# MarcoMeter/endless-memory-gym

Measured on AMD Instinct MI355X. Metric: env steps/sec (aggregate), higher is better.
Workload: dtype u8; 1 GPU; MortarMayhem-Grid-v0, 65536 envs/GPU x 1 GPU, 84x84x3 obs (u8_xyc), same-step auto-reset, uniform random actions generated on device; env_id=MortarMayhem-Grid-v0, envs_per_gpu=65536, envs_total=65536, parallelism=env-sharded x1, no data-path collective

## Files before the change

### endless-memory-gym_amd/csrc/mg_api.hip

```cpp
#include <algorithm>
#include <chrono>
#include <cstddef>
#include <map>
#include <mutex>

#include "mg_family.hpp"
#include "mg_lab.hpp"
using mg::lab_env;

namespace mg {
static thread_local std::string g_last_error;
void set_error(const std::string& msg) { g_last_error = msg; }
}

struct mg_env {
    mg::Family* fam = nullptr;
    int device = 0;
    int num_envs = 0;
    int variant = 0, family = 0;
    bool started = false;
    std::string id;
    int obs_format = MG_OBS_U8_XYC;
    float* vec_dev = nullptr;
    float* vec_dev_caller = nullptr;
    int prof_stride = 0;
    struct Single {
        bool open = false;
        char *host = nullptr, *dev = nullptr;
        size_t bytes = 0;
        size_t o_action = 0, o_seed = 0, o_obs = 0, o_vec = 0, o_reward32 = 0, o_reward = 0, o_done = 0, o_gt32 = 0, o_gt = 0, o_ep_reward = 0,
               o_ep_length = 0, o_aux = 0, o_flag = 0;
        uint32_t ticket = 0;
    } single;
};

namespace {
constexpr size_t INFO_SIZE_MIN = offsetof(mg_info_buffers, final_obs_dev);
mg_info_buffers read_info(const mg_info_buffers* info) {
    mg_info_buffers ib;
    memset(&ib, 0, sizeof(ib));
    if (!info) return ib;
    const size_t sz = info->struct_size;
    constexpr size_t INFO_SIZE_MAX = sizeof(mg_info_buffers) + 16 * sizeof(void*);
    if (sz < INFO_SIZE_MIN || sz > INFO_SIZE_MAX || sz % sizeof(void*) != 0)
        throw std::runtime_error("mg_step: mg_info_buffers.struct_size = " + std::to_string(sz) + " is not a layout of include/memgym.h (" +
                                 std::to_string(sizeof(mg_info_buffers)) + " in this build); set it to sizeof(mg_info_buffers)");
    memcpy(&ib, info, sz < sizeof(ib) ? sz : sizeof(ib));
    ib.struct_size = sizeof(ib);
    return ib;
}

struct StateHeader {
    char magic[8];
    uint32_t version, num_envs;
    uint64_t payload, id_hash;
    uint8_t pad[32];
};
static_assert(sizeof(StateHeader) == 64, "state header is 64 bytes");
uint64_t fnv1a(const std::string& s) {
    uint64_t h = 1469598103934665603ull;
    for (unsigned char c : s) h = (h ^ c) * 1099511628211ull;
    return h;
}

struct DeviceGuard {
    int prev = -1;
    explicit DeviceGuard(int device) {
        MG_HIP(hipGetDevice(&prev));
        if (prev != device) MG_HIP(hipSetDevice(device));
        else prev = -1;
    }
    ~DeviceGuard() {
        if (prev >= 0) (void)hipSetDevice(prev);
    }
};

template <typename F>
int guarded(mg_env* env, F&& f) {
    try {
        if (!env || !env->fam) {
            mg::set_error("null handle");
            return -1;
        }
        DeviceGuard guard(env->device);
        f();
        return 0;
    } catch (const mg::OptionError& e) {
        mg::set_error(e.msg);
        return e.code;
    } catch (const std::exception& e) {
        mg::set_error(e.what());
        return -1;
    }
}
}

namespace {
mg::Family* make_family(int family, int variant, int n) {
    if (family == 0) return mg::make_mortar(variant, n);
    if (family == 1) return mg::make_spot(variant, n);
    return mg::make_mystery(variant, n);
}
void destroy_family(mg_env* e) {
    if (e->single.host) {
        if (e->vec_dev && e->vec_dev == (float*)(e->single.dev + e->single.o_vec)) e->vec_dev = e->vec_dev_caller;
        (void)hipHostFree(e->single.host);
        e->single = mg_env::Single();
    }
    delete e->fam;
    e->fam = nullptr;
}
size_t obs_bytes_of(int f) {
    const size_t elem = f == MG_OBS_F32_CYX ? 4 : ((f == MG_OBS_F16_CYX || f == MG_OBS_BF16_CYX) ? 2 : 1);
    return elem * 84 * 84 * 3;
}
}

extern "C" {

const char* mg_last_error(void) { return mg::g_last_error.c_str(); }

int mg_create(const char* env_id, int32_t num_envs, int device, mg_env** out) {
    try {
        if (!env_id || !out || num_envs < 1) {
            mg::set_error("mg_create: bad arguments");
            return -1;
        }
        DeviceGuard guard(device);
        std::string id(env_id);
        int family = -1, variant = 0;
        if (id == "MortarMayhem-Grid-v0") { family = 0; variant = 0; }
        else if (id == "MortarMayhem-v0") { family = 0; variant = 1; }
        else if (id == "Endless-MortarMayhem-v0") { family = 0; variant = 2; }
        else if (id == "MortarMayhemB-Grid-v0") { family = 0; variant = 3; }
        else if (id == "MortarMayhemB-v0") { family = 0; variant = 4; }
        else if (id == "Endless-SearingSpotlights-v0") { family = 1; variant = 1; }
        else if (id == "SearingSpotlights-v0") { family = 1; variant = 0; }
        else if (id == "MysteryPath-v0") { family = 2; variant = 0; }
        else if (id == "Endless-MysteryPath-v0") { family = 2; variant = 1; }
        else if (id == "MysteryPath-Grid-v0") { family = 2; variant = 2; }
        else {
            mg::set_error("mg_create: environment id not available in this build: " + id);
            return -5;
        }
        mg_env* e = new mg_env();
        e->device = device;
        e->num_envs = num_envs;
        e->id = id;
        e->family = family;
        e->variant = variant;
        try {
            e->fam = make_family(family, variant, num_envs);
        } catch (...) {
            delete e;
            throw;
        }
        *out = e;
        return 0;
    } catch (const std::exception& e) {
        mg::set_error(e.what());
        return -1;
    }
}

void mg_destroy(mg_env* env) {
    if (!env) return;
    int prev = -1;
    (void)hipGetDevice(&prev);
    (void)hipSetDevice(env->device);
    (void)hipDeviceSynchronize();
    destroy_family(env);
    delete env;
    if (prev >= 0) (void)hipSetDevice(prev);
}

int32_t mg_num_envs(const mg_env* env) { return env ? env->num_envs : 0; }
int32_t mg_action_dim(const mg_env* env) { return env ? env->fam->action_dim() : 0; }
int32_t mg_gt_dim(const mg_env* env) { return env ? env->fam->gt_dim() : 0; }
int32_t mg_vec_dim(const mg_env* env) { return env ? env->fam->vec_dim() : 0; }
int mg_bind_vector_obs(mg_env* env, float* vec_dev) {
    return guarded(env, [&] {
        if (env->fam->vec_dim() == 0 && vec_dev) throw std::runtime_error("mg_bind_vector_obs: this env id has no vector observation");
        env->vec_dev = env->vec_dev_caller = vec_dev;
        env->fam->bind_vector_obs(vec_dev);
    });
}
const char* mg_info_name(const mg_env* env, int k) { return env ? env->fam->info_name(k) : nullptr; }

int mg_set_option(mg_env* env, const char* key, const double* values, int n) {
    return guarded(env, [&] {
        if (!key || !values || n < 1) throw mg::OptionError{-3, "mg_set_option: bad arguments"};
        env->fam->set_option(key, values, n);
    });
}

int mg_set_option_set(mg_env* env, int set_id, const char* key, const double* values, int n) {
    return guarded(env, [&] {
        if (!key || !values || n < 1) throw mg::OptionError{-3, "mg_set_option_set: bad arguments"};
        if (set_id < 0 || set_id >= MG_MAX_OPTION_SETS) throw mg::OptionError{-3, "mg_set_option_set: set index out of range"};
        env->fam->set_option_set(set_id, key, values, n);
    });
}

int mg_bind_option_sets(mg_env* env, const int32_t* set_of_dev) {
    return guarded(env, [&] {
        env->fam->bind_option_sets(set_of_dev);
    });
}

int mg_set_capacity(mg_env* env, const char* what, int64_t value) {
    return guarded(env, [&] {
        if (!what) throw mg::OptionError{-3, "mg_set_capacity: NULL"};
        if (env->started) throw std::runtime_error("mg_set_capacity: before the first mg_reset / mg_set_state");
        env->fam->set_capacity(what, value);
    });
}
int64_t mg_capacity(mg_env* env, const char* what) {
    int64_t v = -1;
    const int rc = guarded(env, [&] {
        if (!what) throw mg::OptionError{-3, "mg_capacity: NULL"};
        v = env->fam->capacity(what);
    });
    return rc == 0 ? v : -1;
}

int mg_set_obs_format(mg_env* env, int format) {
    return guarded(env, [&] {
        if (format != MG_OBS_U8_XYC && format != MG_OBS_F32_CYX && format != MG_OBS_F16_CYX && format != MG_OBS_BF16_CYX)
            throw mg::OptionError{-3, "mg_set_obs_format: unknown format"};
        env->obs_format = env->fam->obs_format = format;
    });
}

size_t mg_obs_bytes(const mg_env* env) {
    if (!env) return 0;
    return obs_bytes_of(env->obs_format);
}

int mg_reset(mg_env* env, const int64_t* seeds_dev, const uint8_t* mask_dev, void* obs_dev, float* gt_dev, void* stream) {
    return guarded(env, [&] {
        if (!obs_dev) throw std::runtime_error("mg_reset: obs_dev is NULL");
        env->fam->reset(seeds_dev, mask_dev, obs_dev, gt_dev, (hipStream_t)stream);
        env->started = true;
    });
}

int mg_render(mg_env* env, void* obs_dev, void* stream) {
    return guarded(env, [&] {
        if (!obs_dev) throw std::runtime_error("mg_render: obs_dev is NULL");
        env->fam->raster_only(obs_dev, nullptr, (hipStream_t)stream);
    });
}

typedef uint32_t row_vec16 __attribute__((ext_vector_type(4)));
constexpr int COPY_CHUNK = 16;
__global__ __launch_bounds__(256) void copy_rows_kernel(const uint8_t* __restrict__ flags, const row_vec16* __restrict__ src, row_vec16* __restrict__ dst,
                                                      int n, int vec_per_row) {
    const int tid = threadIdx.x;
    for (int base = blockIdx.x * COPY_CHUNK; base < n; base += gridDim.x * COPY_CHUNK) {
        const int e = base + (tid & (COPY_CHUNK - 1));
        uint32_t m = (uint32_t)__builtin_amdgcn_readfirstlane((int)(uint32_t)__ballot(e < n && flags[e] != 0)) & ((1u << COPY_CHUNK) - 1u);
        while (m) {
            const size_t row = (size_t)(base + __builtin_ctz(m)) * (size_t)vec_per_row;
            m &= m - 1;
            for (int q0 = 0; q0 < vec_per_row; q0 += 6 * 256) {
                row_vec16 v[6];
#pragma unroll
                for (int k = 0; k < 6; ++k) {
                    const int q = q0 + tid + 256 * k;
                    if (q < vec_per_row) v[k] = src[row + q];
                }
#pragma unroll
                for (int k = 0; k < 6; ++k) {
                    const int q = q0 + tid + 256 * k;
                    if (q < vec_per_row) dst[row + q] = v[k];
                }
            }
        }
    }
}

namespace {
__global__ __launch_bounds__(256) void debug_stretch_kernel(const uint8_t* __restrict__ frames, uint8_t* __restrict__ out, int n) {
    const size_t total = (size_t)n * 336 * 336;
    for (size_t p = (size_t)blockIdx.x * blockDim.x + threadIdx.x; p < total; p += (size_t)gridDim.x * blockDim.x) {
        const int x = (int)(p % 336), y = (int)((p / 336) % 336);
        const size_t e = p / (336 * 336);
        const uint8_t* src = frames + e * MG_OBS_BYTES + ((size_t)(x >> 2) * 84 + (y >> 2)) * 3;
        uint8_t* dst = out + p * 3;
        dst[0] = src[0];
        dst[1] = src[1];
        dst[2] = src[2];
    }
}
}

int mg_render_debug(mg_env* env, uint8_t* rgb_dev, void* stream) {
    return guarded(env, [&] {
        if (!rgb_dev) throw std::runtime_error("mg_render_debug: rgb_dev is NULL");
        hipStream_t st = (hipStream_t)stream;
        uint8_t* frames = nullptr;
        MG_HIP(hipMalloc((void**)&frames, (size_t)env->num_envs * MG_OBS_BYTES));
        try {
            env->fam->sync_state();
            env->fam->raster_debug(frames, st);
            const size_t total = (size_t)env->num_envs * 336 * 336;
            const unsigned grid = (unsigned)std::min<size_t>((total + 255) / 256, 65536);
            hipLaunchKernelGGL(debug_stretch_kernel, dim3(grid), dim3(256), 0, st, frames, rgb_dev, env->num_envs);
            MG_HIP(hipGetLastError());
            MG_HIP(hipStreamSynchronize(st));
        } catch (...) {
            (void)hipFree(frames);
            throw;
        }
        MG_HIP(hipFree(frames));
    });
}

int mg_step(mg_env* env, const int32_t* actions_dev, void* obs_dev, float* reward_dev, uint8_t* done_dev, float* gt_dev,
            const mg_info_buffers* info, int autoreset, void* stream) {
    return guarded(env, [&] {
        if (!actions_dev || !obs_dev || !reward_dev || !done_dev) throw std::runtime_error("mg_step: NULL buffer");
        hipStream_t st = (hipStream_t)stream;
        const mg_info_buffers ib = read_info(info);
        mg::Family* f = env->fam;
        if (autoreset && ib.final_obs_dev && !(mg::sparse_masked_raster() && f->keeps_final_obs(st))) {
            f->step(actions_dev, obs_dev, reward_dev, done_dev, gt_dev, &ib, 0, st);
            if (mg::sparse_masked_raster()) {
                const int n = env->num_envs, vec_per_row = (int)(mg_obs_bytes(env) / 16);
                hipLaunchKernelGGL(copy_rows_kernel, dim3(std::min((n + COPY_CHUNK - 1) / COPY_CHUNK, 16384)), dim3(256), 0, st, done_dev, (const row_vec16*)obs_dev,
                                   (row_vec16*)ib.final_obs_dev, n, vec_per_row);
                MG_HIP(hipGetLastError());
            } else f->raster_only(ib.final_obs_dev, done_dev, st);
            f->reset(nullptr, done_dev, obs_dev, gt_dev, st);
        } else {
            f->step(actions_dev, obs_dev, reward_dev, done_dev, gt_dev, &ib, autoreset, st);
        }
        if (ib.gt64_dev) f->ground_truth64(ib.gt64_dev, st);
    });
}

int mg_ground_truth64(mg_env* env, double* gt64_dev, void* stream) {
    return guarded(env, [&] {
        if (!env->fam->gt_dim()) return;
        if (!gt64_dev) throw std::runtime_error("mg_ground_truth64: gt64_dev is NULL");
        env->fam->sync_state();
        env->fam->ground_truth64(gt64_dev, (hipStream_t)stream);
    });
}

}
namespace {
void single_wait(mg_env::Single& S, hipStream_t st, bool armed = false) {
    static bool use_flag = true;
    if (use_flag) {
        const uint32_t want = armed ? S.ticket : ++S.ticket;
        if (armed || hipStreamWriteValue32(st, S.dev + S.o_flag, want, 0) == hipSuccess) {
            volatile uint32_t* flag = (volatile uint32_t*)(S.host + S.o_flag);
            const auto t0 = std::chrono::steady_clock::now();
            for (uint32_t spins = 0;; ++spins) {
                if (__atomic_load_n(flag, __ATOMIC_ACQUIRE) == want) return;
                __builtin_ia32_pause();
                if ((spins & 1023u) == 1023u && std::chrono::steady_clock::now() - t0 > std::chrono::milliseconds(50)) break;
            }
        } else {
            (void)hipGetLastError();
            use_flag = false;
        }
    }
    MG_HIP(hipStreamSynchronize(st));
}
}
extern "C" {
int mg_single_open(mg_env* env, mg_single_io* io) {
    return guarded(env, [&] {
        if (!io || io->struct_size != sizeof(mg_single_io)) throw std::runtime_error("mg_single_open: set io->struct_size = sizeof(mg_single_io)");
        if (env->num_envs != 1) throw std::runtime_error("mg_single_open: the handle must hold exactly one instance");
        mg_env::Single& S = env->single;
        if (!S.open) {
            size_t o = 0;
            auto take = [&](size_t bytes) { const size_t at = o; o = (o + bytes + 255) & ~(size_t)255; return at; };
            S.o_action = take(8); S.o_seed = take(8);
            S.o_obs = take(84 * 84 * 3 * 4);
            S.o_vec = take(sizeof(float) * 256);
            S.o_reward32 = take(4); S.o_reward = take(8); S.o_done = take(1);
            S.o_gt32 = take(sizeof(float) * 8); S.o_gt = take(sizeof(double) * 8);
            S.o_ep_reward = take(8); S.o_ep_length = take(4); S.o_aux = take(sizeof(float) * MG_INFO_SLOTS * 64);
            S.o_flag = take(4);
            S.bytes = o;
            MG_HIP(hipHostMalloc((void**)&S.host, S.bytes, hipHostMallocMapped | hipHostMallocCoherent));
            memset(S.host, 0, S.bytes);
            MG_HIP(hipHostGetDevicePointer((void**)&S.dev, S.host, 0));
            S.open = true;
        }
        if (env->fam->vec_dim()) {
            env->vec_dev = (float*)(S.dev + S.o_vec);
            env->fam->bind_vector_obs(env->vec_dev);
        }
        io->obs = S.host + S.o_obs;
        io->vec = env->fam->vec_dim() ? (float*)(S.host + S.o_vec) : nullptr;
        io->reward = (double*)(S.host + S.o_reward);
        io->done = (uint8_t*)(S.host + S.o_done);
        io->gt = (double*)(S.host + S.o_gt);
        io->ep_reward = (double*)(S.host + S.o_ep_reward);
        io->ep_length = (int32_t*)(S.host + S.o_ep_length);
        for (int k = 0; k < MG_INFO_SLOTS; ++k) io->aux[k] = (float*)(S.host + S.o_aux + 256 * k);
    });
}

int mg_single_reset(mg_env* env, int64_t seed, int has_seed, void* stream) {
    return guarded(env, [&] {
        mg_env::Single& S = env->single;
        if (!S.open) throw std::runtime_error("mg_single_reset: mg_single_open first");
        hipStream_t st = (hipStream_t)stream;
        *(int64_t*)(S.host + S.o_seed) = seed;
        mg::Family* f = env->fam;
        f->reset(has_seed ? (const int64_t*)(S.dev + S.o_seed) : nullptr, nullptr, S.dev + S.o_obs, f->gt_dim() ? (float*)(S.dev + S.o_gt32) : nullptr, st);
        f->ground_truth64((double*)(S.dev + S.o_gt), st);
        env->started = true;
        single_wait(S, st);
    });
}

int mg_single_step(mg_env* env, int32_t a0, int32_t a1, void* stream) {
    int flags = 0;
    const int rc = guarded(env, [&] {
        mg_env::Single& S = env->single;
        if (!S.open) throw std::runtime_error("mg_single_step: mg_single_open first");
        hipStream_t st = (hipStream_t)stream;
        int32_t* act = (int32_t*)(S.host + S.o_action);
        act[0] = a0;
        act[1] = a1;
        mg_info_buffers ib;
        memset(&ib, 0, sizeof(ib));
        ib.struct_size = sizeof(ib);
        ib.ep_reward_dev = (double*)(S.dev + S.o_ep_reward);
        ib.ep_length_dev = (int32_t*)(S.dev + S.o_ep_length);
        for (int k = 0; k < MG_INFO_SLOTS; ++k) ib.aux_dev[k] = (float*)(S.dev + S.o_aux + 256 * k);
        ib.reward64_dev = (double*)(S.dev + S.o_reward);
        mg::Family* f = env->fam;
        const bool armed = f->arm_done_flag((uint32_t*)(S.dev + S.o_flag), S.ticket + 1);
        if (armed) ++S.ticket;
        f->step((const int32_t*)(S.dev + S.o_action), S.dev + S.o_obs, (float*)(S.dev + S.o_reward32), (uint8_t*)(S.dev + S.o_done),
                f->gt_dim() ? (float*)(S.dev + S.o_gt32) : nullptr, &ib, 0, st);
        f->ground_truth64((double*)(S.dev + S.o_gt), st);
        single_wait(S, st, armed);
        flags = f->peek_errors();
    });
    return rc != 0 ? rc : flags;
}

size_t mg_state_size(const mg_env* env) {
    if (!env) return 0;
    size_t t = sizeof(StateHeader);
    for (auto& b : env->fam->state_blobs()) t += b.second;
    return t;
}

int mg_get_state(mg_env* env, void* host_buf, size_t size) {
    return guarded(env, [&] {
        if (!host_buf || size < mg_state_size(env)) throw std::runtime_error("mg_get_state: buffer too small");
        MG_HIP(hipDeviceSynchronize());
        env->fam->sync_state();
        StateHeader h;
        memset(&h, 0, sizeof(h));
        memcpy(h.magic, "MGSTATE1", 8);
        h.version = MG_STATE_VERSION;
        h.num_envs = (uint32_t)env->num_envs;
        h.payload = mg_state_size(env) - sizeof(StateHeader);
        h.id_hash = fnv1a(env->id);
        memcpy(host_buf, &h, sizeof(h));
        char* p = (char*)host_buf + sizeof(StateHeader);
        for (auto& b : env->fam->state_blobs()) {
            MG_HIP(hipMemcpy(p, b.first, b.second, hipMemcpyDeviceToHost));
            p += b.second;
        }
    });
}

int mg_set_state(mg_env* env, const void* host_buf, size_t size) {
    return guarded(env, [&] {
        if (!host_buf || size < sizeof(StateHeader)) throw std::runtime_error("mg_set_state: buffer too small for a state header");
        StateHeader h;
        memcpy(&h, host_buf, sizeof(h));
        if (memcmp(h.magic, "MGSTATE1", 8) != 0) throw std::runtime_error("mg_set_state: not a memgym state blob (bad magic)");
        if (h.version != MG_STATE_VERSION)
            throw std::runtime_error("mg_set_state: state version " + std::to_string(h.version) + ", this library reads version " +
                                     std::to_string(MG_STATE_VERSION));
        if (h.id_hash != fnv1a(env->id)) throw std::runtime_error("mg_set_state: the blob belongs to another env id than " + env->id);
        if (h.num_envs != (uint32_t)env->num_envs)
            throw std::runtime_error("mg_set_state: the blob holds " + std::to_string(h.num_envs) + " instances, the handle " +
                                     std::to_string(env->num_envs));
        if (h.payload != mg_state_size(env) - sizeof(StateHeader) || size < mg_state_size(env))
            throw std::runtime_error("mg_set_state: payload size differs from this handle's state");
        MG_HIP(hipDeviceSynchronize());
        const char* p = (const char*)host_buf + sizeof(StateHeader);
        for (auto& b : env->fam->state_blobs()) {
            MG_HIP(hipMemcpy(b.first, p, b.second, hipMemcpyHostToDevice));
            p += b.second;
        }
        env->fam->on_state_loaded();
        env->started = true;
    });
}

int mg_set_profiling(mg_env* env, int on) {
    return guarded(env, [&] {
        env->prof_stride = on < 0 ? 0 : on;
        env->fam->prof.stride = env->prof_stride;
        env->fam->prof.count[0] = env->fam->prof.count[1] = 0;
    });
}

int mg_get_profile(mg_env* env, int kind, double* total_ms, int64_t* launches) {
    return guarded(env, [&] {
        if (kind < 0 || kind > 1 || !total_ms || !launches) throw std::runtime_error("mg_get_profile: bad arguments");
        env->fam->prof.collect(kind, total_ms, launches);
    });
}

int mg_poll_errors(mg_env* env, int* flags) {
    return guarded(env, [&] {
        if (!flags) throw std::runtime_error("mg_poll_errors: NULL");
        MG_HIP(hipDeviceSynchronize());
        *flags = env->fam->poll_errors();
    });
}

int mg_peek_errors(mg_env* env, int* flags) {
    return guarded(env, [&] {
        if (!flags) throw std::runtime_error("mg_peek_errors: NULL");
        *flags = env->fam->peek_errors();
    });
}

int mg_enable_peer_access(int device, int peer_device) {
    try {
        int prev = 0;
        MG_HIP(hipGetDevice(&prev));
        struct Restore {
            int d;
            ~Restore() { (void)hipSetDevice(d); }
        } restore{prev};
        if (device == peer_device) return 0;
        int can = 0;
        MG_HIP(hipDeviceCanAccessPeer(&can, device, peer_device));
        if (!can) {
            mg::set_error("device " + std::to_string(device) + " has no peer access to device " + std::to_string(peer_device));
            return -1;
        }
        MG_HIP(hipSetDevice(device));
        hipError_t e = hipDeviceEnablePeerAccess(peer_device, 0);
        if (e != hipSuccess && e != hipErrorPeerAccessAlreadyEnabled) {
            (void)hipGetLastError();
            mg::set_error(std::string("hipDeviceEnablePeerAccess: ") + hipGetErrorString(e));
            return -1;
        }
        (void)hipGetLastError();
        return 0;
    } catch (const std::exception& e) {
        mg::set_error(e.what());
        return -1;
    }
}

int mg_debug_counter(mg_env* env, const char* name, int64_t* value) {
    return guarded(env, [&] {
        if (!name || !value) throw std::runtime_error("mg_debug_counter: NULL");
        MG_HIP(hipDeviceSynchronize());
        if (!env->fam->debug_counter(name, value)) throw std::runtime_error(std::string("mg_debug_counter: no counter named ") + name + " for " + env->id);
    });
}

int mg_debug_rng(mg_env* env, int32_t i, uint64_t* out) {
    return guarded(env, [&] {
        if (i < 0 || i >= env->num_envs) throw std::runtime_error("mg_debug_rng: index out of range");
        MG_HIP(hipDeviceSynchronize());
        env->fam->sync_state();
        env->fam->debug_rng(i, out);
    });
}

}
```

### endless-memory-gym_amd/csrc/mg_family.hpp

```cpp
#pragma once
#include <hip/hip_runtime.h>

#include <cstdint>
#include <cstdio>
#include <cstring>
#include <stdexcept>
#include <string>
#include <vector>

#include "../../include/memgym.h"
#include "mg_lab.hpp"
#include "mg_device.hpp"

namespace mg {

void set_error(const std::string& msg);
static_assert(MG_MAX_OPTION_SETS == 8, "set_index() (mg_device.hpp) masks an instance's set index with 7");

#define MG_HIP(expr)                                                                                 \
    do {                                                                                             \
        hipError_t e_ = (expr);                                                                      \
        if (e_ != hipSuccess)                                                                        \
            throw std::runtime_error(std::string(#expr) + " failed: " + hipGetErrorString(e_));      \
    } while (0)

struct ErrorWord {
    int* host = nullptr;
    int* dev = nullptr;
    ErrorWord() {}
    ErrorWord(const ErrorWord&) = delete;
    ErrorWord& operator=(const ErrorWord&) = delete;
    ~ErrorWord() {
        if (host) (void)hipHostFree(host);
    }
    void alloc() {
        MG_HIP(hipHostMalloc((void**)&host, 64, hipHostMallocMapped | hipHostMallocCoherent));
        *host = 0;
        MG_HIP(hipHostGetDevicePointer((void**)&dev, host, 0));
    }
    int peek() const { return __atomic_load_n(host, __ATOMIC_ACQUIRE); }
    int take() { return __atomic_exchange_n(host, 0, __ATOMIC_ACQ_REL); }
};

#ifdef __HIPCC__
__device__ __forceinline__ void raise_error(int* err, int bit) {
    __hip_atomic_fetch_or(err, bit, __ATOMIC_RELAXED, __HIP_MEMORY_SCOPE_SYSTEM);
}
constexpr int ERR_QUEUE_OVERFLOW = 64;
__device__ __forceinline__ void queue_push(int* queue, int* counter, int cap, int value, int* err) {
    const int slot = atomicAdd(counter, 1);
    if (__builtin_expect(slot < cap, 1)) queue[slot] = value;
    else raise_error(err, ERR_QUEUE_OVERFLOW);
}
__device__ __forceinline__ int queue_count(const int* counter, int cap) {
    const int c = *counter;
    return c < cap ? c : cap;
}
#endif

template <typename T>
struct DevArray {
    T* p = nullptr;
    size_t n = 0;
    DevArray() {}
    DevArray(const DevArray&) = delete;
    DevArray& operator=(const DevArray&) = delete;
    ~DevArray() { release(); }
    void release() {
        if (p) (void)hipFree(p);
        p = nullptr;
        n = 0;
    }
    void alloc(size_t count, bool zero = true) {
        release();
        n = count;
        MG_HIP(hipMalloc((void**)&p, sizeof(T) * (count ? count : 1)));
        if (zero) MG_HIP(hipMemset(p, 0, sizeof(T) * (count ? count : 1)));
    }
    void upload(const std::vector<T>& v) {
        alloc(v.size(), false);
        MG_HIP(hipMemcpy(p, v.data(), sizeof(T) * v.size(), hipMemcpyHostToDevice));
    }
    size_t bytes() const { return sizeof(T) * n; }
};

struct RngStore {
    DevArray<uint64_t> s_hi, s_lo, i_hi, i_lo, buf;
    void alloc(size_t n) { s_hi.alloc(n); s_lo.alloc(n); i_hi.alloc(n); i_lo.alloc(n); buf.alloc(n); }
    RngSoA view() { return RngSoA{s_hi.p, s_lo.p, i_hi.p, i_lo.p, buf.p}; }
    void blobs(std::vector<std::pair<void*, size_t>>& v) {
        v.push_back({s_hi.p, s_hi.bytes()}); v.push_back({s_lo.p, s_lo.bytes()}); v.push_back({i_hi.p, i_hi.bytes()});
        v.push_back({i_lo.p, i_lo.bytes()}); v.push_back({buf.p, buf.bytes()});
    }
    void debug(int i, uint64_t out[6]) {
        uint64_t b;
        MG_HIP(hipMemcpy(&out[0], s_hi.p + i, 8, hipMemcpyDeviceToHost));
        MG_HIP(hipMemcpy(&out[1], s_lo.p + i, 8, hipMemcpyDeviceToHost));
        MG_HIP(hipMemcpy(&out[2], i_hi.p + i, 8, hipMemcpyDeviceToHost));
        MG_HIP(hipMemcpy(&out[3], i_lo.p + i, 8, hipMemcpyDeviceToHost));
        MG_HIP(hipMemcpy(&b, buf.p + i, 8, hipMemcpyDeviceToHost));
        out[4] = (b >> 32) & 1;
        out[5] = b & 0xFFFFFFFFull;
    }
};

struct OptListStore {
    DevArray<int32_t> ext;
    std::vector<int> host;
    int max(const OptList& l) const {
        int m = 0;
        if (!host.empty() || l.ext) {
            for (int x : host) m = x > m ? x : m;
            return m;
        }
        for (int k = 0; k < l.n && k < OPT_INLINE; ++k) {
            const int x = (int)((l.w[k >> 2] >> (8 * (k & 3))) & 0xFFu);
            m = x > m ? x : m;
        }
        return m;
    }
    void set(OptList& l, const std::vector<int>& v) {
        host = v;
        l.n = (int)v.size();
        for (int j = 0; j < OPT_INLINE / 4; ++j) l.w[j] = 0u;
        l.ext = nullptr;
        bool bytes = true;
        for (int x : v) bytes = bytes && x >= 0 && x <= 255;
        for (int k = 0; bytes && k < l.n && k < OPT_INLINE; ++k) l.w[k >> 2] |= (uint32_t)(v[k] & 0xFF) << (8 * (k & 3));
        if (l.n > OPT_INLINE || !bytes) {
            std::vector<int32_t> b(v.begin(), v.end());
            MG_HIP(hipDeviceSynchronize());
            ext.upload(b);
            l.ext = ext.p;
        }
    }
};

struct OptionError {
    int code;
    std::string msg;
};

struct KernelProfile {
    int stride = 0;
    uint64_t count[2] = {0, 0};
    bool live[2] = {false, false};
    std::vector<std::pair<hipEvent_t, hipEvent_t>> ev[2];
    void begin(int kind, hipStream_t s) {
        live[kind] = stride > 0 && (count[kind]++ % (uint64_t)stride) == 0;
        if (!live[kind]) return;
        hipEvent_t a, b;
        MG_HIP(hipEventCreate(&a));
        MG_HIP(hipEventCreate(&b));
        MG_HIP(hipEventRecord(a, s));
        ev[kind].push_back({a, b});
    }
    void end(int kind, hipStream_t s) {
        if (!live[kind]) return;
        MG_HIP(hipEventRecord(ev[kind].back().second, s));
    }
    void collect(int kind, double* ms, int64_t* launches) {
        double t = 0;
        for (auto& p : ev[kind]) {
            MG_HIP(hipEventSynchronize(p.second));
            float f = 0;
            MG_HIP(hipEventElapsedTime(&f, p.first, p.second));
            t += f;
            (void)hipEventDestroy(p.first);
            (void)hipEventDestroy(p.second);
        }
        *ms = t;
        *launches = (int64_t)ev[kind].size();
        ev[kind].clear();
    }
};

class Family {
   public:
    KernelProfile prof;
    void end_logic(hipStream_t s) { prof.end(0, s); }
    int obs_format = MG_OBS_U8_XYC;
    virtual ~Family() {}
    virtual int action_dim() const = 0;
    virtual int gt_dim() const = 0;
    virtual bool arm_done_flag(uint32_t* , uint32_t ) { return false; }
    virtual void set_capacity(const std::string& what, int64_t) { throw OptionError{-2, "this env id has no capacity named " + what}; }
    virtual int64_t capacity(const std::string& what) const { throw OptionError{-2, "this env id has no capacity named " + what}; }
    virtual int vec_dim() const { return 0; }
    virtual void bind_vector_obs(float* ) {}
    virtual const char* info_name(int k) const = 0;
    virtual void set_option(const std::string& key, const double* v, int n) = 0;
    virtual void set_option_set(int set, const std::string& key, const double* v, int n) {
        if (set != 0) throw OptionError{-3, "this env id has no per-instance option sets in this build (use one handle per option set)"};
        set_option(key, v, n);
    }
    virtual void bind_option_sets(const int32_t* set_of_dev) {
        if (set_of_dev) throw OptionError{-3, "this env id has no per-instance option sets in this build (use one handle per option set)"};
    }
    virtual void reset(const int64_t* seeds, const uint8_t* mask, void* obs, float* gt, hipStream_t s) = 0;
    virtual void step(const int32_t* actions, void* obs, float* reward, uint8_t* done, float* gt,
                      const mg_info_buffers* info, int autoreset, hipStream_t s) = 0;
    virtual void raster_only(void* obs, const uint8_t* only, hipStream_t s) = 0;
    virtual bool keeps_final_obs(hipStream_t ) { return false; }
    virtual void raster_debug(void* frames, hipStream_t s) = 0;
    virtual std::vector<std::pair<void*, size_t>> state_blobs() = 0;
    virtual void on_state_loaded() {}
    virtual void sync_state() {}
    virtual void debug_rng(int i, uint64_t out[6]) = 0;
    virtual void ground_truth64(double* , hipStream_t ) {}
    virtual int poll_errors() { return 0; }
    virtual int peek_errors() { return 0; }
    virtual bool debug_counter(const std::string& , int64_t* ) { return false; }
};

Family* make_mortar(int variant, int num_envs);
Family* make_spot(int endless, int num_envs);
Family* make_mystery(int variant, int num_envs);

inline int step_block(int shipped) {
    static const int forced = [] {
        const char* e = lab_env("MEMGYM_STEP_BLOCK");
        const int v = e ? atoi(e) : 0;
        return (v == 64 || v == 128 || v == 256) ? v : 0;
    }();
    return forced ? forced : shipped;
}

inline int to_int_checked(double v, const char* key) {
    int i = (int)v;
    if ((double)i != v) throw OptionError{-3, std::string("option ") + key + " must be integral"};
    return i;
}

}
```

### endless-memory-gym_amd/csrc/mg_mortar.hip

```cpp
#include <memory>

#include "mg_atlas_v1.hpp"
#include "mg_device.hpp"
#include "mg_family.hpp"
#include "mg_lab.hpp"
#include "mg_raster_v1.hpp"
#include "mg_stamps.hpp"

namespace mg {
using namespace v1;

enum { V_GRID = 0, V_FREE = 1, V_ENDLESS = 2 };

struct MortarParams {
    int variant, N, allowed, visual_feedback, max_steps, initial_count;
    int taskb;
    int cmd_cap;
    int arena_x0, tile;
    int radius, sprite_dim;
    int glyph_x0;
    int v_axis_i, v_diag_i;
    int off_lo, off_hi;
    double v_axis, v_diag;
    OptList command_count, show_dur, show_delay, expl_dur, expl_delay;
    double r_fail, r_succ, r_ep_succ, r_new;
};

struct __attribute__((aligned(16))) MortarState {
    int16_t ax, ay;
    int16_t disp_x, disp_y;
    uint8_t rot8 : 3;
    uint8_t disp_is_agent : 1;
    uint8_t tiles_on : 1;
    uint8_t disp_sprite;
    int8_t tx, ty;
    int8_t nx, ny;
    uint16_t num_cmds, cur_cmd;
    uint16_t vis_pos, vis_len, vis_base;
    uint16_t cmd_steps, verify_step;
    uint16_t show_dur, show_delay, expl_dur, expl_delay;
    uint8_t gx, gy;
    int32_t ep_len, t, total_completed;
    uint32_t dbg_pops;
    double ep_sum;
};
static_assert(sizeof(MortarState) == 64, "MortarState must be 64 bytes");

struct __attribute__((aligned(16))) MortarDesc {
    int16_t sx, sy;
    uint16_t tmpl;
    uint8_t sprite;
    uint8_t glyph;
    int16_t glyph_x0;
    int16_t ring_x, ring_y;
    uint8_t ring_on;
    uint8_t epoch;
};
static_assert(sizeof(MortarDesc) == 16, "MortarDesc must be 16 bytes");
constexpr int STAMP_SPRITE0 = 0, STAMP_GLYPH0 = 8, STAMP_RING = 18;

struct MortarComposer {
    typedef MortarDesc Desc;
    static __device__ __forceinline__ bool skip(const Desc* dp) { return dp->tmpl == 0xFFFF; }
    static __device__ __forceinline__ void compose(const Desc* dp, const RasterCtx& R) {
        const Desc& d = *dp;
#if defined(MG_LAB_NO_TEMPLATE) && MG_LAB_NO_TEMPLATE == 2
#elif defined(MG_LAB_NO_TEMPLATE)
        fill_clear(R);
#else
        fill_template(R, d.tmpl);
#endif
        __syncthreads();
#ifndef MG_LAB_NO_STAMPS
        if (d.sprite != 0xFF) stamp(R, STAMP_SPRITE0 + d.sprite, d.sx, d.sy);
        if (d.glyph < 9) {
            __syncthreads();
            stamp(R, STAMP_GLYPH0 + d.glyph, d.glyph_x0, d.glyph_x0);
        }
#endif
    }
};

struct MortarDebugComposer {
    typedef MortarDesc Desc;
    static __device__ __forceinline__ bool skip(const Desc*) { return false; }
    static __device__ __forceinline__ void compose(const Desc* dp, const RasterCtx& R) {
        MortarComposer::compose(dp, R);
        __syncthreads();
        if (dp->ring_on) stamp(R, STAMP_RING, dp->ring_x, dp->ring_y);
    }
};

constexpr uint32_t pack_deltas(const int (&v)[9]) {
    uint32_t m = 0;
    for (int c = 0; c < 9; ++c) m |= (uint32_t)(v[c] + 1) << (2 * c);
    return m;
}
constexpr int kDxHost[9] = {1, 0, -1, 0, 0, 1, 1, -1, -1}, kDyHost[9] = {0, 1, 0, -1, 0, 1, -1, 1, -1};
constexpr uint32_t CMD_DX_BITS = pack_deltas(kDxHost), CMD_DY_BITS = pack_deltas(kDyHost);
__device__ __forceinline__ int cmd_dx(int c) { return (int)((CMD_DX_BITS >> (2 * c)) & 3u) - 1; }
__device__ __forceinline__ int cmd_dy(int c) { return (int)((CMD_DY_BITS >> (2 * c)) & 3u) - 1; }

__device__ __forceinline__ int floordiv(int a, int b) {
    int q = a / b;
    return (a % b != 0 && a < 0) ? q - 1 : q;
}
__device__ __forceinline__ int mod6(int a) { return ((a % 6) + 6) % 6; }
__device__ __forceinline__ int round_haz(double v) { return v >= 0 ? (int)floor(v + 0.5) : -(int)floor(-v + 0.5); }

__constant__ int8_t kCmdOneHot[9] = {1, 4, 2, 3, 0, 5, 6, 7, 8};
constexpr int VEC_DIM = 180;

__device__ void mortar_reset(const MortarParams& P, MortarState& s, Pcg& g, uint8_t* cmds, MortarDesc& d, float* gt, float* vec) {
    if (s.disp_sprite != 0xFF && s.disp_is_agent) {
        s.disp_x = s.ax;
        s.disp_y = s.ay;
        s.disp_is_agent = 0;
    }
    int half = P.tile / 2;
    int tile_id = g.integers(0, P.N * P.N);
    int cx = P.arena_x0 + P.tile * (tile_id / P.N) + half;
    int cy = P.arena_x0 + P.tile * (tile_id % P.N) + half;
    if (P.variant == V_ENDLESS || (P.taskb && P.variant == V_FREE)) {
        cx += g.integers(P.off_lo, P.off_hi);
        cy += g.integers(P.off_lo, P.off_hi);
    }
    s.ax = (int16_t)cx;
    s.ay = (int16_t)cy;
    s.rot8 = 0;
    int nx = floordiv(cx - P.arena_x0, P.tile), ny = floordiv(cy - P.arena_x0, P.tile);
    s.nx = (int8_t)nx;
    s.ny = (int8_t)ny;
    s.gx = (uint8_t)nx;
    s.gy = (uint8_t)ny;

    int n;
    if (P.variant == V_ENDLESS) {
        n = P.initial_count;
        for (int i = 0; i < n; ++i) cmds[i] = (uint8_t)g.integers(0, P.allowed);
    } else {
        n = choice(g, P.command_count);
        int px = nx, py = ny;
        for (int i = 0; i < n; ++i) {
            uint32_t valid = 0;
#pragma unroll
            for (int c = 0; c < 9; ++c) {
                const int qx = px + cmd_dx(c), qy = py + cmd_dy(c);
                if (c < P.allowed && qx >= 0 && qx < P.N && qy >= 0 && qy < P.N) valid |= 1u << c;
            }
            const int pick = g.integers(0, __popc(valid));
            uint32_t m = valid;
            for (int k = 0; k < pick; ++k) m &= m - 1;
            const int c = __ffs(m) - 1;
            cmds[i] = (uint8_t)c;
            px += cmd_dx(c);
            py += cmd_dy(c);
        }
    }
    s.num_cmds = (uint16_t)n;
    if (P.taskb) {
        s.show_dur = s.show_delay = 0;
    } else {
        s.show_dur = (uint16_t)choice(g, P.show_dur);
        s.show_delay = (uint16_t)choice(g, P.show_delay);
    }
    s.vis_len = (uint16_t)(n * (s.show_dur + s.show_delay));
    s.vis_base = 0;
    s.vis_pos = 1;
    s.dbg_pops = 0;
    int first = cmds[0];
    uint8_t glyph = s.show_dur > 0 ? (uint8_t)first : (uint8_t)9;
    if (P.variant == V_ENDLESS) {
        s.tx = (int8_t)mod6(nx + cmd_dx(first));
        s.ty = (int8_t)mod6(ny + cmd_dy(first));
    } else {
        s.tx = (int8_t)(nx + cmd_dx(first));
        s.ty = (int8_t)(ny + cmd_dy(first));
    }
    s.cur_cmd = 0;
    s.cmd_steps = 0;
    s.verify_step = 0;
    s.total_completed = 0;
    s.tiles_on = 0;
    s.t = 0;
    s.ep_len = 0;
    s.ep_sum = 0.0;
    s.expl_dur = (uint16_t)choice(g, P.expl_dur);
    s.expl_delay = (uint16_t)choice(g, P.expl_delay);

    d.tmpl = 0;
    d.sprite = 0;
    d.sx = (int16_t)(cx - P.sprite_dim / 2);
    d.sy = (int16_t)(cy - P.sprite_dim / 2);
    d.glyph = glyph;
    if (gt) {
        gt[0] = (float)(s.tx / 5.0);
        gt[1] = (float)(s.ty / 5.0);
    }
    if (vec) {
        for (int k = 0; k < VEC_DIM; ++k) vec[k] = 0.0f;
        for (int c = 0; c < n && c < VEC_DIM / 9; ++c) vec[9 * c + kCmdOneHot[cmds[c]]] = 1.0f;
    }
}

struct MortarIO {
    MortarState* state;
    uint8_t* cmds;
    RngSoA rng;
    MortarDesc* desc;
    float* vec;
    int* err;
    const MortarParams* sets;
    const int32_t* set_of;
};
constexpr int ERR_CMD_OVERFLOW = 32;

template <bool PS>
__global__ __launch_bounds__(256) void mortar_reset_kernel(MortarParams P0, int n, MortarIO io, const int64_t* seeds,
                                                           const uint8_t* mask, float* gt) {
    int i = blockIdx.x * blockDim.x + threadIdx.x;
    if (i >= n) return;
    const MortarParams& P = PS ? io.sets[set_index(io.set_of, i)] : P0;
    MortarDesc d;
    memset(&d, 0, sizeof(d));
    d.glyph_x0 = (int16_t)P.glyph_x0;
    if (mask && !mask[i]) {
        d.tmpl = 0xFFFF;
        io.desc[i] = d;
        return;
    }
    Pcg g;
    if (seeds) g.seed((uint64_t)seeds[i]);
    else g.load(io.rng, i);
    MortarState s = io.state[i];
    mortar_reset(P, s, g, io.cmds + (size_t)i * P.cmd_cap, d, gt ? gt + 2 * i : nullptr, io.vec ? io.vec + (size_t)i * VEC_DIM : nullptr);
    io.state[i] = s;
    g.store(io.rng, i);
    io.desc[i] = d;
}

__global__ __launch_bounds__(256) void mortar_init_kernel(int n, MortarState* state) {
    int i = blockIdx.x * blockDim.x + threadIdx.x;
    if (i >= n) return;
    MortarState s;
    memset(&s, 0, sizeof(s));
    s.disp_sprite = 0xFF;
    state[i] = s;
}

struct MortarStepArgs {
    MortarParams P;
    int n;
    MortarIO io;
    const int32_t* actions;
    float* reward_out;
    uint8_t* done_out;
    float* gt;
    mg_info_buffers info;
    int autoreset;
    MortarDesc* tdesc;
};

template <bool FUSED, bool CLAIM = false, bool PS = false, bool FINAL = false>
__device__ __forceinline__ void mortar_step_body(int i, const MortarStepArgs& a, uint32_t epoch, uint32_t* claim_word = nullptr,
                                                 uint32_t ticket = 0u) {
    uint32_t claimed_by = 0u;
    if constexpr (CLAIM) {
        claimed_by = ticket + 1u;
        if ((threadIdx.x & 63) == 0) claimed_by = __hip_atomic_exchange(claim_word, ticket, __ATOMIC_RELAXED, __HIP_MEMORY_SCOPE_AGENT);
    }
    const MortarIO& io = a.io;
    const MortarParams& P = PS ? io.sets[set_index(io.set_of, i)] : a.P;
    const int32_t* const actions = a.actions;
    float* const reward_out = a.reward_out;
    uint8_t* const done_out = a.done_out;
    float* const gt = a.gt;
    const mg_info_buffers& info = a.info;
    const int autoreset = a.autoreset;
    const bool one_action = P.variant == V_GRID;
    int act0 = actions[one_action ? i : 2 * i], act1 = actions[one_action ? i : 2 * i + 1];
    Pcg g;
    bool rng_loaded = !FUSED;
    if constexpr (!FUSED) g.load(io.rng, i);
    MortarState s = io.state[i];
    asm volatile("" : "+v"(act0), "+v"(act1));
    if constexpr (!FUSED) g.pin();
    if constexpr (CLAIM) {
        asm volatile("" : "+v"(claimed_by));
        if ((uint32_t)__builtin_amdgcn_readfirstlane((int)claimed_by) == ticket) return;
    }
    uint8_t* cmds = io.cmds + (size_t)i * P.cmd_cap;
    double reward = 0.0;
    bool done = false, cap = false;
    int success = 0;
    uint8_t glyph = 0xFF;
    bool rng_used = false;

    if (s.vis_pos < s.vis_len) {
        int period = s.show_dur + s.show_delay;
        int k = s.vis_pos / period, w = s.vis_pos % period;
        glyph = (w < s.show_dur) ? cmds[s.vis_base + k] : (uint8_t)9;
        s.vis_pos++;
        if (P.variant != V_ENDLESS || s.disp_sprite == 0xFF) {
            s.disp_sprite = 0;
            s.disp_is_agent = 1;
        }
    } else {
        int ax = s.ax, ay = s.ay;
        if (P.variant == V_GRID) {
            int a = act0;
            int rot = s.rot8 * 45;
            if (a == 1) rot = (rot + 90) % 360;
            if (a == 2) rot = (rot + 270) % 360;
            int gx = s.gx, gy = s.gy;
            if (a == 3) {
                int face = rot / 90;
                if (face == 0) { if (gy > 0) gy--; }
                else if (face == 3) { if (gx < P.N - 1) gx++; }
                else if (face == 2) { if (gy < P.N - 1) gy++; }
                else { if (gx > 0) gx--; }
                ax = P.arena_x0 + P.tile * gx + P.tile / 2;
                ay = P.arena_x0 + P.tile * gy + P.tile / 2;
            }
            s.gx = (uint8_t)gx;
            s.gy = (uint8_t)gy;
            s.rot8 = (uint8_t)(rot / 45);
        } else {
            int a0 = act0, a1 = act1;
            int dxs = a0 == 1 ? -1 : (a0 == 2 ? 1 : 0), dys = a1 == 1 ? -1 : (a1 == 2 ? 1 : 0);
            int rot = s.rot8 * 45;
            if (a0 == 1) rot = 90;
            if (a0 == 2) rot = 270;
            if (a1 == 1) rot = 0;
            if (a1 == 2) rot = 180;
            if (dxs < 0 && dys < 0) rot = 45;
            if (dxs < 0 && dys > 0) rot = 135;
            if (dxs > 0 && dys < 0) rot = 315;
            if (dxs > 0 && dys > 0) rot = 225;
            s.rot8 = (uint8_t)(rot / 45);
            bool diag = dxs != 0 && dys != 0;
            if (P.variant == V_FREE) {
                int v = diag ? P.v_diag_i : P.v_axis_i;
                ax += dxs * v;
                ay += dys * v;
                int lo = P.arena_x0 + P.radius, hi = P.arena_x0 + P.tile * P.N - P.radius;
                ax = ax > hi ? hi : ax;
                ax = ax < lo ? lo : ax;
                ay = ay > hi ? hi : ay;
                ay = ay < lo ? lo : ay;
            } else {
                double v = diag ? P.v_diag : P.v_axis;
                ax = round_haz((double)ax + dxs * v);
                ay = round_haz((double)ay + dys * v);
                double left = P.arena_x0, right = P.arena_x0 + P.tile * P.N, off = P.radius * 0.5;
                double x = ax, y = ay;
                if (x > right + off) x = left - off;
                if (x < left - off) x = right + off;
                if (y > right + off) y = left - off;
                if (y < left - off) y = right + off;
                ax = round_haz(x);
                ay = round_haz(y);
            }
        }
        s.ax = (int16_t)ax;
        s.ay = (int16_t)ay;
        s.disp_sprite = s.rot8;
        s.disp_is_agent = 1;
        int nx = floordiv(ax - P.arena_x0, P.tile), ny = floordiv(ay - P.arena_x0, P.tile);
        s.nx = (int8_t)nx;
        s.ny = (int8_t)ny;
        bool on_target = (nx == s.tx) && (ny == s.ty);

        bool verify = (s.cmd_steps % s.expl_delay == 0) && s.cmd_steps > 0;
        if (verify && !s.tiles_on) {
            if (s.cur_cmd < s.num_cmds) {
                s.cur_cmd++;
                s.tiles_on = 1;
                if (on_target) {
                    reward += P.r_succ;
                    if (P.variant == V_ENDLESS) {
                        s.total_completed++;
                        if (s.cur_cmd == s.num_cmds) reward += P.r_new;
                    }
                } else {
                    done = true;
                    reward += P.r_fail;
                }
            }
            if (s.cur_cmd >= s.num_cmds) {
                if (P.variant == V_ENDLESS) {
                    if (!rng_loaded) g.load(io.rng, i);
                    rng_loaded = true;
                    rng_used = true;
                    int nc = g.integers(0, P.allowed);
                    if (s.num_cmds < P.cmd_cap) {
                        cmds[s.num_cmds] = (uint8_t)nc;
                        s.vis_base = s.num_cmds;
                        s.num_cmds++;
                    } else {
                        raise_error(io.err, ERR_CMD_OVERFLOW);
                        done = true;
                        cap = true;
                        s.vis_base = (uint16_t)(s.num_cmds - 1);
                    }
                    s.cur_cmd = 0;
                    s.verify_step = 0;
                    s.vis_pos = 0;
                    s.vis_len = (uint16_t)(s.show_dur + s.show_delay);
                    s.dbg_pops = 0;
                } else {
                    done = true;
                    success = 1;
                    reward += P.r_ep_succ;
                }
            }
            s.cmd_steps = 1;
        }
        if (s.tiles_on) {
            if (s.verify_step % s.expl_dur == 0 && s.verify_step > 0) {
                s.tiles_on = 0;
                s.verify_step = 0;
                if (s.cur_cmd < s.num_cmds) {
                    int c = cmds[s.cur_cmd];
                    if (P.variant == V_ENDLESS) {
                        s.tx = (int8_t)mod6(s.tx + cmd_dx(c));
                        s.ty = (int8_t)mod6(s.ty + cmd_dy(c));
                    } else {
                        s.tx = (int8_t)(s.tx + cmd_dx(c));
                        s.ty = (int8_t)(s.ty + cmd_dy(c));
                    }
                }
            } else {
                if (!on_target) {
                    done = true;
                    reward = P.r_fail;
                }
                s.verify_step++;
            }
        } else {
            s.cmd_steps++;
        }
    }

    if (P.variant == V_ENDLESS) {
        s.t++;
        if (s.t == P.max_steps) done = true;
    }
    s.ep_sum += reward;
    s.ep_len++;

    if (done) {
        if (info.ep_reward_dev) info.ep_reward_dev[i] = s.ep_sum;
        if (info.ep_length_dev) info.ep_length_dev[i] = s.ep_len;
        if (P.variant == V_ENDLESS) {
            if (info.aux_dev[0]) info.aux_dev[0][i] = (float)s.total_completed;
            if (info.aux_dev[1]) info.aux_dev[1][i] = (float)(s.num_cmds > 1 ? s.num_cmds - 1 : 0);
        } else {
            if (info.aux_dev[0]) info.aux_dev[0][i] = (float)success;
            if (info.aux_dev[1]) info.aux_dev[1][i] = (float)((double)((int)s.cur_cmd - 1 + success) / (double)s.num_cmds);
        }
    }
    reward_out[i] = (float)reward;
    if (info.reward64_dev) info.reward64_dev[i] = reward;
    done_out[i] = done ? 1 : 0;
    if (info.capacity_dev) info.capacity_dev[i] = cap ? 1 : 0;

    MortarDesc d;
    memset(&d, 0, sizeof(d));
    d.glyph_x0 = (int16_t)P.glyph_x0;
    if (done && autoreset) {
        if constexpr (FINAL) {
            MortarDesc td;
            memset(&td, 0, sizeof(td));
            td.glyph_x0 = (int16_t)P.glyph_x0;
            const int tcx = s.disp_is_agent ? s.ax : s.disp_x, tcy = s.disp_is_agent ? s.ay : s.disp_y;
            td.sx = (int16_t)(tcx - P.sprite_dim / 2);
            td.sy = (int16_t)(tcy - P.sprite_dim / 2);
            td.sprite = s.disp_sprite;
            td.glyph = glyph;
            td.tmpl = (uint16_t)((s.tiles_on && P.visual_feedback) ? 1 + s.tx * P.N + s.ty : 0);
            uint32_t tw[4];
            memcpy(tw, &td, sizeof(tw));
            uint32_t* tdst = reinterpret_cast<uint32_t*>(&a.tdesc[i]);
            __hip_atomic_store(tdst + 0, tw[0], __ATOMIC_RELAXED, __HIP_MEMORY_SCOPE_AGENT);
            __hip_atomic_store(tdst + 1, tw[1], __ATOMIC_RELAXED, __HIP_MEMORY_SCOPE_AGENT);
            __hip_atomic_store(tdst + 2, tw[2], __ATOMIC_RELAXED, __HIP_MEMORY_SCOPE_AGENT);
            __hip_atomic_store(tdst + 3, tw[3], __ATOMIC_RELAXED, __HIP_MEMORY_SCOPE_AGENT);
        }
        if (!rng_loaded) g.load(io.rng, i);
        rng_loaded = true;
        rng_used = true;
        mortar_reset(P, s, g, cmds, d, (gt && P.variant == V_ENDLESS) ? gt + 2 * i : nullptr, io.vec ? io.vec + (size_t)i * VEC_DIM : nullptr);
        if constexpr (FINAL) d.ring_on = 1;
    } else {
        int cx = s.disp_is_agent ? s.ax : s.disp_x, cy = s.disp_is_agent ? s.ay : s.disp_y;
        d.sx = (int16_t)(cx - P.sprite_dim / 2);
        d.sy = (int16_t)(cy - P.sprite_dim / 2);
        d.sprite = s.disp_sprite;
        d.glyph = glyph;
        d.tmpl = (uint16_t)((s.tiles_on && P.visual_feedback) ? 1 + s.tx * P.N + s.ty : 0);
        if (gt && P.variant == V_ENDLESS) {
            gt[2 * i] = (float)(s.tx / 5.0);
            gt[2 * i + 1] = (float)(s.ty / 5.0);
        }
    }
    if (rng_used) g.store(io.rng, i);
    io.state[i] = s;
    if constexpr (FUSED) {
        d.epoch = (uint8_t)epoch;
        uint32_t w[4];
        memcpy(w, &d, sizeof(w));
        uint32_t* dst = reinterpret_cast<uint32_t*>(&io.desc[i]);
        __hip_atomic_store(dst + 0, w[0], __ATOMIC_RELAXED, __HIP_MEMORY_SCOPE_AGENT);
        __hip_atomic_store(dst + 1, w[1], __ATOMIC_RELAXED, __HIP_MEMORY_SCOPE_AGENT);
        __hip_atomic_store(dst + 2, w[2], __ATOMIC_RELAXED, __HIP_MEMORY_SCOPE_AGENT);
        asm volatile("s_waitcnt vmcnt(0)" ::: "memory");
        __hip_atomic_store(dst + 3, w[3], __ATOMIC_RELAXED, __HIP_MEMORY_SCOPE_AGENT);
    } else {
        io.desc[i] = d;
    }
}

template <bool PS>
__global__ __launch_bounds__(256) void mortar_step_kernel(MortarStepArgs a) {
    const int i = blockIdx.x * blockDim.x + threadIdx.x;
    if (i < a.n) mortar_step_body<false, false, PS>(i, a, 0u);
}

#define MG_KERNARG_AS __attribute__((address_space(4)))
constexpr unsigned long long RESCUE_AFTER_TICKS = 20000;
template <bool DONE_FLAG, bool FINAL = false>
__global__ __launch_bounds__(256, 7) void mortar_step_raster_kernel(MortarStepArgs a, int logic_wgs, int logic_base, uint32_t epoch,
                                                                    uint32_t ticket, uint32_t* claims, uint32_t* rescues,
                                                                    RasterAtlas A, void* __restrict__ obs, uint32_t* done_flag, uint32_t done_ticket) {
    const int n = a.n;
    const int tid = threadIdx.x, lane = tid & 63;
    const int rel = (int)blockIdx.x - logic_base;
    const bool is_logic = rel >= 0 && rel < logic_wgs;
    auto claim = [&](int q) -> bool {
        uint32_t old = 0;
        if (lane == 0) old = __hip_atomic_exchange(claims + q, ticket, __ATOMIC_RELAXED, __HIP_MEMORY_SCOPE_AGENT);
        return (uint32_t)__builtin_amdgcn_readfirstlane((int)old) != ticket;
    };
    if (is_logic) {
        const int q = rel * 4 + (tid >> 6), i = q * 64 + lane;
#if defined(MG_LABV) && MG_LABV >= 1
        if (i < n) mortar_step_body<true, false, false, FINAL>(i, a, epoch);
#else
        if (i < n) mortar_step_body<true, true, false, FINAL>(i, a, epoch, claims + q, ticket);
#endif
        return;
    }
    extern __shared__ __attribute__((aligned(16))) uint8_t smem[];
    RasterCtx R;
    R.frame = smem;
    R.mask = reinterpret_cast<uint32_t*>(smem + FRAME_BYTES);
    R.A = A;
    R.T = A.tables;
    R.tid = tid;
    const int stride = (int)gridDim.x - logic_wgs;
    for (int v = (int)blockIdx.x < logic_base ? (int)blockIdx.x : (int)blockIdx.x - logic_wgs; v < n; v += stride) {
        const int env = xcd_grouped_frame(v, n);
        const uint32_t* src = reinterpret_cast<const uint32_t*>(a.io.desc + env);
        uint32_t w[4];
        bool tried = false;
        unsigned long long t0 = 0;
        for (int polls = 0;; ++polls) {
            w[3] = (uint32_t)__builtin_amdgcn_readfirstlane((int)__hip_atomic_load(src + 3, __ATOMIC_RELAXED, __HIP_MEMORY_SCOPE_AGENT));
            if ((w[3] >> 24) == epoch) break;
#if defined(MG_LABV) && MG_LABV >= 2
            if (false) {
#else
            if (polls == 0) t0 = wall_clock64();
            if (!tried && (polls & 15) == 15 && wall_clock64() - t0 >= RESCUE_AFTER_TICKS) {
#endif
                tried = true;
                if (claim(env >> 6)) {
                    const MortarStepArgs MG_KERNARG_AS* ka = (const MortarStepArgs MG_KERNARG_AS*)__builtin_amdgcn_kernarg_segment_ptr();
                    asm volatile("" : "+s"(ka));
                    int i = (env >> 6) * 64 + lane;
                    asm volatile("" : "+v"(i));
                    if (i < n) mortar_step_body<true, false, false, FINAL>(i, *(const MortarStepArgs*)ka, epoch);
                    if (lane == 0) atomicAdd(rescues, 1u);
                    continue;
                }
            }
            __builtin_amdgcn_s_sleep(4);
        }
        asm volatile("" ::: "memory");
        w[0] = __hip_atomic_load(src + 0, __ATOMIC_RELAXED, __HIP_MEMORY_SCOPE_AGENT);
        w[1] = __hip_atomic_load(src + 1, __ATOMIC_RELAXED, __HIP_MEMORY_SCOPE_AGENT);
        w[2] = __hip_atomic_load(src + 2, __ATOMIC_RELAXED, __HIP_MEMORY_SCOPE_AGENT);
        MortarDesc d;
        memcpy(&d, w, sizeof(d));
        if constexpr (FINAL) {
            if (d.ring_on) {
                const uint32_t* tsrc = reinterpret_cast<const uint32_t*>(a.tdesc + env);
                uint32_t tw[4];
#pragma unroll
                for (int k = 0; k < 4; ++k) tw[k] = __hip_atomic_load(tsrc + k, __ATOMIC_RELAXED, __HIP_MEMORY_SCOPE_AGENT);
                MortarDesc td;
                memcpy(&td, tw, sizeof(td));
                int tt = tid;
                asm volatile("" : "+v"(tt));
                R.tid = tt;
                MortarComposer::compose(&td, R);
                __syncthreads();
                store_frame<MG_OBS_U8_XYC, false>(smem, a.info.final_obs_dev, env, tt);
                __syncthreads();
            }
        }
        if (MortarComposer::skip(&d)) continue;
        int t = tid;
        asm volatile("" : "+v"(t));
        R.tid = t;
        MortarComposer::compose(&d, R);
        __syncthreads();
        store_frame<MG_OBS_U8_XYC, false>(smem, obs, env, t);
        __syncthreads();
    }
    if constexpr (DONE_FLAG) {
        __builtin_amdgcn_fence(__ATOMIC_RELEASE, "");
        __syncthreads();
        if (tid == 0) __hip_atomic_store(done_flag, done_ticket, __ATOMIC_RELAXED, __HIP_MEMORY_SCOPE_SYSTEM);
    }
}

__global__ __launch_bounds__(256) void mortar_gt64_kernel(int n, const MortarState* state, double* out) {
    const int i = blockIdx.x * blockDim.x + threadIdx.x;
    if (i >= n) return;
    const MortarState s = state[i];
    out[2 * i] = s.tx / 5.0;
    out[2 * i + 1] = s.ty / 5.0;
}

__global__ __launch_bounds__(256) void mortar_debug_desc_kernel(MortarParams P0, int n, MortarIO io, MortarDesc* out) {
    const int i = blockIdx.x * blockDim.x + threadIdx.x;
    if (i >= n) return;
    const MortarParams& P = io.set_of ? io.sets[set_index(io.set_of, i)] : P0;
    const MortarState s = io.state[i];
    const uint8_t* cmds = io.cmds + (size_t)i * P.cmd_cap;
    MortarDesc d = io.desc[i];
    {
        const bool have = s.disp_sprite != 0xFF;
        const int cx = (have && !s.disp_is_agent) ? s.disp_x : s.ax, cy = (have && !s.disp_is_agent) ? s.disp_y : s.ay;
        d.sx = (int16_t)(cx - P.sprite_dim / 2);
        d.sy = (int16_t)(cy - P.sprite_dim / 2);
        d.sprite = have ? s.disp_sprite : (uint8_t)0;
        d.tmpl = (uint16_t)((s.tiles_on && P.visual_feedback) ? 1 + s.tx * P.N + s.ty : 0);
        d.glyph_x0 = (int16_t)P.glyph_x0;
    }
    d.glyph = 0xFF;
    if (s.vis_pos < s.vis_len) {
        const int idx = (int)s.dbg_pops, period = s.show_dur + s.show_delay;
        io.state[i].dbg_pops = s.dbg_pops + 1;
        if (idx >= 0 && idx < (int)s.vis_len && period > 0) {
            const int k = idx / period, w = idx % period;
            d.glyph = (w < s.show_dur) ? cmds[s.vis_base + k] : (uint8_t)9;
        }
    }
    const int r = P.tile / 2;
    d.ring_x = (int16_t)(P.arena_x0 + P.tile * s.tx + P.tile / 2 - r);
    d.ring_y = (int16_t)(P.arena_x0 + P.tile * s.ty + P.tile / 2 - r);
    d.ring_on = 1;
    out[i] = d;
}

static const double SCALE = 0.25;

class MortarFamily : public Family {
   public:
    MortarFamily(int variant_id, int n) : opt_(one_set()), P_(opt_[0]->P), n_(n) {
        memset(&P_, 0, sizeof(P_));
        const int variant = variant_id >= 3 ? variant_id - 3 : variant_id;
        P_.variant = variant;
        P_.taskb = variant_id >= 3;
        agent_scale_ = 1.0 * SCALE;
        agent_speed_ = 12.0 * SCALE;
        P_.N = variant == V_ENDLESS ? 6 : 5;
        P_.allowed = variant == V_GRID ? 5 : 9;
        P_.visual_feedback = 1;
        P_.max_steps = -1;
        P_.initial_count = 1;
        P_.cmd_cap = variant == V_ENDLESS ? 512 : 32;
        if (variant == V_ENDLESS) {
            const int cap = lab_int("MEMGYM_EMM_CMD_CAP", 0);
            if (cap >= 4 && cap <= 512) P_.cmd_cap = cap;
        }
        MortarOpt& O = *opt_[0];
        O.st_command_count.set(P_.command_count, {10});
        O.st_show_dur.set(P_.show_dur, {3});
        O.st_show_delay.set(P_.show_delay, {1});
        O.st_expl_dur.set(P_.expl_dur, {variant == V_GRID ? 2 : 6});
        O.st_expl_delay.set(P_.expl_delay, {variant == V_GRID ? 6 : 18});
        P_.r_fail = 0.0;
        P_.r_succ = 0.1;
        P_.r_ep_succ = 0.0;
        P_.r_new = 0.0;
        state_.alloc(n);
        cmds_.alloc((size_t)n * P_.cmd_cap);
        desc_.alloc(n);
        tdesc_.alloc(n);
        rng_.alloc(n);
        err_.alloc();
        claims_.alloc((size_t)((n + 255) / 256) * 4);
        rescues_.alloc(1);
        sets_dev_.alloc(MG_MAX_OPTION_SETS);
        hipLaunchKernelGGL(mortar_init_kernel, dim3((n + 255) / 256), dim3(256), 0, 0, n, state_.p);
        MG_HIP(hipDeviceSynchronize());
        rebuild();
        defaults_ = P_;
    }

    void set_capacity(const std::string& what, int64_t v) override {
        if (!(P_.variant == V_ENDLESS && what == "commands")) return Family::set_capacity(what, v);
        if (v < 4 || v > 32768) throw OptionError{-3, "commands: 4 .. 32,768"};
        if (seeded_) throw std::runtime_error("mg_set_capacity: before the first reset");
        if (2 * P_.initial_count > v) throw OptionError{-3, "commands: below twice the initial_command_count in force"};
        MG_HIP(hipDeviceSynchronize());
        P_.cmd_cap = (int)v;
        cmds_.alloc((size_t)n_ * P_.cmd_cap);
        for (size_t k = 1; k < opt_.size(); ++k) copy_geometry(opt_[k]->P, P_);
        copy_geometry(defaults_, P_);
        sets_dirty_ = true;
    }
    int64_t capacity(const std::string& what) const override {
        if (P_.variant == V_ENDLESS && what == "commands") return P_.cmd_cap;
        return Family::capacity(what);
    }
    bool arm_done_flag(uint32_t* flag_dev, uint32_t ticket) override {
        if (!(n_ == 1 && obs_format == MG_OBS_U8_XYC && fuse_step() && !per_set() && gt_dim() == 0 && !dirty_)) return false;
        flag_dev_ = flag_dev;
        flag_ticket_ = ticket;
        flag_armed_ = true;
        return true;
    }
    int action_dim() const override { return P_.variant == V_GRID ? 1 : 2; }
    int gt_dim() const override { return P_.variant == V_ENDLESS ? 2 : 0; }
    int vec_dim() const override { return P_.taskb ? VEC_DIM : 0; }
    void bind_vector_obs(float* dev) override { vec_ = dev; }
    const char* info_name(int k) const override {
        if (P_.variant == V_ENDLESS) return k == 0 ? "commands_completed" : (k == 1 ? "max_command_sequence" : nullptr);
        return k == 0 ? "success" : (k == 1 ? "commands_completed" : nullptr);
    }

    void set_option(const std::string& key, const double* v, int n) override { set_option_set(0, key, v, n); }
    void set_option_set(int set, const std::string& key, const double* v, int n) override {
        if (set < 0 || set >= MG_MAX_OPTION_SETS) throw OptionError{-3, "option set index out of range"};
        while ((int)opt_.size() <= set) {
            opt_.emplace_back(new MortarOpt());
            opt_.back()->P = defaults_;
            copy_geometry(opt_.back()->P, P_);
        }
        MortarOpt& O = *opt_[set];
        MortarParams& P = O.P;
        const bool endless = P_.variant == V_ENDLESS;
        auto geometry = [&]() {
            if (set != 0) throw OptionError{-3, "reset parameter " + key + " changes the geometry shared by the handle's instances: it can only be set for all of them (option set 0)"};
        };
        auto scalar_i = [&](int& dst) { dst = to_int_checked(v[0], key.c_str()); };
        auto list = [&](OptList& l, OptListStore& st, int lo, int hi) {
            if (n < 1) throw OptionError{-3, "option " + key + ": an empty list cannot be sampled"};
            std::vector<int> vals(n);
            for (int i = 0; i < n; ++i) {
                vals[i] = to_int_checked(v[i], key.c_str());
                if (vals[i] < lo || vals[i] > hi)
                    throw OptionError{-3, "option " + key + ": value out of the supported range " + std::to_string(lo) + ".." + std::to_string(hi)};
            }
            st.set(l, vals);
        };
        if (key == "agent_scale") { if (set != 0) { if (v[0] != agent_scale_) geometry(); } else { agent_scale_ = v[0]; dirty_ = true; } }
        else if (key == "allowed_commands") {
            int a = to_int_checked(v[0], key.c_str());
            if (a < 4 || a > 9) throw OptionError{-4, "assert 4 <= allowed_commands <= 9"};
            P.allowed = a;
        }
        else if (!P_.taskb && key == "command_show_duration") list(P.show_dur, O.st_show_dur, 1, 65535);
        else if (!P_.taskb && key == "command_show_delay") list(P.show_delay, O.st_show_delay, 0, 65535);
        else if (key == "explosion_duration") list(P.expl_dur, O.st_expl_dur, 1, 65535);
        else if (key == "explosion_delay") list(P.expl_delay, O.st_expl_delay, 1, 65535);
        else if (key == "visual_feedback") P.visual_feedback = v[0] != 0.0;
        else if (key == "reward_command_failure") P.r_fail = v[0];
        else if (key == "reward_command_success") P.r_succ = v[0];
        else if (endless && key == "max_steps") scalar_i(P.max_steps);
        else if (endless && key == "initial_command_count") {
            int c = to_int_checked(v[0], key.c_str());
            if (c < 1 || c > P_.cmd_cap / 2) throw OptionError{-3, "initial_command_count out of the supported range"};
            P.initial_count = c;
        }
        else if (endless && key == "reward_new_command_success") P.r_new = v[0];
        else if (!endless && key == "arena_size") {
            int a = to_int_checked(v[0], key.c_str());
            if (a < 2 || a > 6) throw OptionError{-4, "assert 2 <= arena_size <= 6"};
            if (set != 0 && a != P_.N) geometry();
            if (set == 0 && a != P_.N) {
                P_.N = a;
                dirty_ = true;
            }
        }
        else if (!endless && key == "command_count") list(P.command_count, O.st_command_count, 1, P_.taskb ? VEC_DIM / 9 : P_.cmd_cap);
        else if (!endless && key == "reward_episode_success") P.r_ep_succ = v[0];
        else if (P_.variant != V_GRID && key == "agent_speed") { if (set != 0) { if (v[0] != agent_speed_) geometry(); } else { agent_speed_ = v[0]; dirty_ = true; } }
        else throw OptionError{-2, "unknown reset parameter " + key};
        sets_dirty_ = true;
    }
    void bind_option_sets(const int32_t* set_of_dev) override { set_of_ = set_of_dev; }

    void reset(const int64_t* seeds, const uint8_t* mask, void* obs, float* gt, hipStream_t s) override {
        if (dirty_) rebuild();
        if (!seeds && !seeded_) throw std::runtime_error("reset(seed=None) before any seeded reset");
        for (auto& O : opt_) {
            const long long n_max = P_.variant == V_ENDLESS ? O->P.initial_count : O->st_command_count.max(O->P.command_count);
            if (!P_.taskb && n_max * ((long long)O->st_show_dur.max(O->P.show_dur) + O->st_show_delay.max(O->P.show_delay)) > 65535)
                throw OptionError{-3, "command_count x (command_show_duration + command_show_delay) exceeds the 65,535 entries of this build's display schedule"};
        }
        if (seeds) seeded_ = true;
        upload_sets(s);
        if (per_set())
            hipLaunchKernelGGL(mortar_reset_kernel<true>, dim3((n_ + 255) / 256), dim3(256), 0, s, P_, n_, io(), seeds, mask, gt_dim() ? gt : nullptr);
        else
            hipLaunchKernelGGL(mortar_reset_kernel<false>, dim3((n_ + 255) / 256), dim3(256), 0, s, P_, n_, io(), seeds, mask, gt_dim() ? gt : nullptr);
        if (mask && sparse_masked_raster()) {
            launch_raster_sparse<MortarComposer>(desc_.p, atlas_->dev(), obs, obs_format, n_, s, mask);
            MG_HIP(hipGetLastError());
        } else raster(obs, s);
    }

    void step(const int32_t* actions, void* obs, float* reward, uint8_t* done, float* gt, const mg_info_buffers* info,
              int autoreset, hipStream_t s) override {
        if (dirty_) throw std::runtime_error("options that change geometry need a reset before the next step");
        mg_info_buffers ib;
        memset(&ib, 0, sizeof(ib));
        if (info) ib = *info;
        upload_sets(s);
        const MortarStepArgs sa{P_, n_, io(), actions, reward, done, gt_dim() ? gt : nullptr, ib, autoreset, nullptr};
        if (obs_format == MG_OBS_U8_XYC && fuse_step() && !per_set() && !capturing(s)) {
            epoch_ = epoch_ % 255u + 1u;
            ++ticket_;
            const int logic_wgs = (n_ + 255) / 256;
            const int frames = n_ < raster_grid(n_) ? n_ : raster_grid(n_);
            static const bool logic_last = lab_int("MEMGYM_LAB_LOGIC_LAST", 0) != 0;
            prof.begin(1, s);
            if (flag_armed_ && n_ == 1) {
                hipLaunchKernelGGL(mortar_step_raster_kernel<true>, dim3(logic_wgs + frames), dim3(256), RASTER_LDS, s, sa, logic_wgs,
                                   logic_last ? frames : 0, epoch_, ticket_, claims_.p, rescues_.p, atlas_->dev(), obs, flag_dev_, flag_ticket_);
                flag_armed_ = false;
            } else if (ib.final_obs_dev && autoreset) {
                MortarStepArgs fa = sa;
                fa.tdesc = tdesc_.p;
                hipLaunchKernelGGL((mortar_step_raster_kernel<false, true>), dim3(logic_wgs + frames), dim3(256), RASTER_LDS, s, fa, logic_wgs,
                                   logic_last ? frames : 0, epoch_, ticket_, claims_.p, rescues_.p, atlas_->dev(), obs, (uint32_t*)nullptr, 0u);
            } else {
                hipLaunchKernelGGL(mortar_step_raster_kernel<false>, dim3(logic_wgs + frames), dim3(256), RASTER_LDS, s, sa, logic_wgs,
                                   logic_last ? frames : 0, epoch_, ticket_, claims_.p, rescues_.p, atlas_->dev(), obs, (uint32_t*)nullptr, 0u);
            }
            MG_HIP(hipGetLastError());
            prof.end(1, s);
            return;
        }
        prof.begin(0, s);
        const int sb = step_block(256);
        if (per_set()) hipLaunchKernelGGL(mortar_step_kernel<true>, dim3((n_ + sb - 1) / sb), dim3(sb), 0, s, sa);
        else hipLaunchKernelGGL(mortar_step_kernel<false>, dim3((n_ + sb - 1) / sb), dim3(sb), 0, s, sa);
        end_logic(s);
        prof.begin(1, s);
        raster(obs, s);
        prof.end(1, s);
    }

    std::vector<std::pair<void*, size_t>> state_blobs() override {
        std::vector<std::pair<void*, size_t>> v = {{state_.p, state_.bytes()}, {cmds_.p, cmds_.bytes()}};
        rng_.blobs(v);
        return v;
    }

    void debug_rng(int i, uint64_t out[6]) override { rng_.debug(i, out); }
    void ground_truth64(double* out, hipStream_t s) override {
        if (!gt_dim() || !out) return;
        hipLaunchKernelGGL(mortar_gt64_kernel, dim3((n_ + 255) / 256), dim3(256), 0, s, n_, state_.p, out);
        MG_HIP(hipGetLastError());
    }
    int poll_errors() override {
        MG_HIP(hipDeviceSynchronize());
        return err_.take();
    }
    int peek_errors() override { return err_.peek(); }
    bool debug_counter(const std::string& name, int64_t* out) override {
        if (name == "cmd_list_max" || name == "cmd_list_ge12") {
            std::vector<MortarState> h(n_);
            MG_HIP(hipDeviceSynchronize());
            MG_HIP(hipMemcpy(h.data(), state_.p, sizeof(MortarState) * (size_t)n_, hipMemcpyDeviceToHost));
            int64_t mx = 0, ge = 0;
            for (const MortarState& s : h) {
                mx = s.num_cmds > mx ? s.num_cmds : mx;
                ge += s.num_cmds >= 12;
            }
            *out = name == "cmd_list_max" ? mx : ge;
            return true;
        }
        if (name != "one_launch_rescues") return false;
        uint32_t v = 0;
        MG_HIP(hipMemcpy(&v, rescues_.p, sizeof v, hipMemcpyDeviceToHost));
        *out = (int64_t)v;
        return true;
    }

   private:
    uint32_t* flag_dev_ = nullptr;
    uint32_t flag_ticket_ = 0;
    bool flag_armed_ = false;
    uint32_t ticket_ = 0;
    uint32_t epoch_ = 0;
    static bool fuse_step() {
        static const bool on = lab_int("MEMGYM_MORTAR_FUSE", 1) != 0;
        return on;
    }
    static bool capturing(hipStream_t s) {
        hipStreamCaptureStatus st = hipStreamCaptureStatusNone;
        return hipStreamIsCapturing(s, &st) == hipSuccess && st != hipStreamCaptureStatusNone;
    }
    MortarIO io() {
        MortarIO o;
        o.state = state_.p;
        o.cmds = cmds_.p;
        o.rng = rng_.view();
        o.desc = desc_.p;
        o.vec = vec_;
        o.err = err_.dev;
        o.sets = per_set() ? sets_dev_.p : nullptr;
        o.set_of = per_set() ? set_of_ : nullptr;
        return o;
    }

    void rebuild() {
        int radius = 0;
        std::vector<Stamp> sprites = build_agent_sprites(P_.variant == V_GRID ? 1.0 * SCALE : agent_scale_, &radius);
        std::vector<Stamp> glyphs = build_glyphs(SCALE);
        P_.tile = (int)(56 * SCALE);
        P_.arena_x0 = SCREEN / 2 - ((P_.tile * P_.N) >> 1);
        P_.radius = radius;
        P_.sprite_dim = sprites[0].w;
        double inv = 1.0 / std::sqrt(2.0);
        P_.v_axis = (1.0 / 1.0) * agent_speed_;
        P_.v_diag = inv * agent_speed_;
        P_.v_axis_i = (int)P_.v_axis;
        P_.v_diag_i = (int)P_.v_diag;
        P_.off_lo = (int)(-8 * SCALE);
        P_.off_hi = (int)(8 * SCALE);

        atlas_.reset(new Atlas());
        for (auto& sp : sprites) atlas_->add_stamp(sp);
        for (auto& g : glyphs) atlas_->add_stamp(g);
        {
            const int r = P_.tile / 2;
            Stamp ring_stamp(2 * r, 2 * r);
            circle(ring_stamp, r, r, r, (int)(8 * SCALE), 6);
            atlas_->add_stamp(ring_stamp);
        }
        atlas_->set_templates(build_mortar_templates(P_.N, SCALE, SCREEN));
        atlas_->upload();
        P_.glyph_x0 = (int)((SCREEN / 2) - std::floor(88 * SCALE / 2));
        dirty_ = false;
        for (size_t k = 1; k < opt_.size(); ++k) copy_geometry(opt_[k]->P, P_);
        copy_geometry(defaults_, P_);
        sets_dirty_ = true;
    }

    struct MortarOpt {
        MortarParams P;
        OptListStore st_command_count, st_show_dur, st_show_delay, st_expl_dur, st_expl_delay;
    };
    static std::vector<std::unique_ptr<MortarOpt>> one_set() {
        std::vector<std::unique_ptr<MortarOpt>> v;
        v.emplace_back(new MortarOpt());
        return v;
    }
    static void copy_geometry(MortarParams& d, const MortarParams& s) {
        d.variant = s.variant; d.N = s.N; d.taskb = s.taskb; d.cmd_cap = s.cmd_cap; d.arena_x0 = s.arena_x0; d.tile = s.tile;
        d.radius = s.radius; d.sprite_dim = s.sprite_dim; d.glyph_x0 = s.glyph_x0; d.v_axis_i = s.v_axis_i; d.v_diag_i = s.v_diag_i;
        d.off_lo = s.off_lo; d.off_hi = s.off_hi; d.v_axis = s.v_axis; d.v_diag = s.v_diag;
    }
    bool per_set() const { return set_of_ != nullptr && opt_.size() > 1; }
    void upload_sets(hipStream_t s) {
        if (!per_set() || !sets_dirty_) return;
        MortarParams fresh = defaults_;
        copy_geometry(fresh, P_);
        std::vector<MortarParams> host(MG_MAX_OPTION_SETS, fresh);
        for (size_t k = 0; k < opt_.size(); ++k) host[k] = opt_[k]->P;
        MG_HIP(hipMemcpyAsync(sets_dev_.p, host.data(), sizeof(MortarParams) * host.size(), hipMemcpyHostToDevice, s));
        MG_HIP(hipStreamSynchronize(s));
        sets_dirty_ = false;
    }

    void raster_only(void* obs, const uint8_t* only, hipStream_t s) override {
        launch_raster<MortarComposer>(desc_.p, atlas_->dev(), obs, obs_format, n_, s, only);
        MG_HIP(hipGetLastError());
    }
    bool keeps_final_obs(hipStream_t s) override {
        static const bool wanted = lab_int("MEMGYM_MORTAR_FINAL_FUSED", 1) != 0;
        return wanted && obs_format == MG_OBS_U8_XYC && fuse_step() && !per_set() && !capturing(s) && !(flag_armed_ && n_ == 1);
    }

    void raster(void* obs, hipStream_t s) {
        launch_raster<MortarComposer>(desc_.p, atlas_->dev(), obs, obs_format, n_, s);
        MG_HIP(hipGetLastError());
    }

   public:
    void raster_debug(void* frames, hipStream_t s) override {
        if (dirty_) throw std::runtime_error("options that change geometry need a reset before the next render");
        DevArray<MortarDesc> dbg;
        dbg.alloc(n_, false);
        hipLaunchKernelGGL(mortar_debug_desc_kernel, dim3((n_ + 255) / 256), dim3(256), 0, s, P_, n_, io(), dbg.p);
        launch_raster<MortarDebugComposer>(dbg.p, atlas_->dev(), frames, MG_OBS_U8_XYC, n_, s);
        MG_HIP(hipGetLastError());
        MG_HIP(hipStreamSynchronize(s));
    }

   private:

    std::vector<std::unique_ptr<MortarOpt>> opt_;
    MortarParams& P_;
    MortarParams defaults_;
    const int32_t* set_of_ = nullptr;
    bool sets_dirty_ = true;
    DevArray<MortarParams> sets_dev_;
    int n_;
    std::unique_ptr<Atlas> atlas_;
    double agent_scale_, agent_speed_;
    bool dirty_ = true, seeded_ = false;

   public:
    void on_state_loaded() override { seeded_ = true; }

   private:
    float* vec_ = nullptr;
    DevArray<MortarState> state_;
    DevArray<uint8_t> cmds_;
    DevArray<MortarDesc> desc_, tdesc_;
    RngStore rng_;
    ErrorWord err_;
    DevArray<uint32_t> claims_, rescues_;
};

Family* make_mortar(int variant, int num_envs) { return new MortarFamily(variant, num_envs); }

}

#ifdef MG_LAB
extern "C" int mg_lab_set_window_offsets(const long long* off, int n) {
    long long v[16] = {0};
    for (int i = 0; i < n && i < 16; ++i) v[i] = off[i];
    return hipMemcpyToSymbol(HIP_SYMBOL(mg::v1::g_lab_win_off), v, sizeof v) == hipSuccess ? 0 : -1;
}
#endif
```

### endless-memory-gym_amd/csrc/mg_placement.hip

```cpp
#include <algorithm>
#include <chrono>
#include <cmath>
#include <map>
#include <mutex>
#include <vector>

#include "mg_family.hpp"
#include "mg_lab.hpp"
using mg::lab_env;

namespace {

constexpr size_t MiB = 1ull << 20, GiB = 1ull << 30;
constexpr size_t PIECE = 304 * MiB;
constexpr int FILL_STEP = 32;
constexpr int PROBE_GRID = 14336;
static const double PRIOR_SAME_TBPS = lab_env("MEMGYM_OBS_SAME_TBPS") ? atof(lab_env("MEMGYM_OBS_SAME_TBPS")) : 5.35;
static const double PRIOR_CROSS_TBPS = lab_env("MEMGYM_OBS_CROSS_TBPS") ? atof(lab_env("MEMGYM_OBS_CROSS_TBPS")) : 5.85;
struct Calib {
    std::vector<double> seen;
    bool relative = false;
    double same_t = PRIOR_SAME_TBPS, cross_t = PRIOR_CROSS_TBPS;
    void observe(double t) {
        if (seen.size() < 256) seen.push_back(t);
        std::vector<double> v(seen);
        std::sort(v.begin(), v.end());
        relative = false;
        same_t = PRIOR_SAME_TBPS;
        cross_t = PRIOR_CROSS_TBPS;
        if (v.size() < 4 || v.back() < 1.15 * v.front()) return;
        size_t cut = 0;
        double gap = 0;
        for (size_t k = 2; k + 2 <= v.size(); ++k)
            if (v[k] / v[k - 1] > gap) {
                gap = v[k] / v[k - 1];
                cut = k;
            }
        if (cut == 0 || gap < 1.07) return;
        const double mid = std::sqrt(v[cut - 1] * v[cut]);
        relative = true;
        same_t = std::max(v[cut - 1] * 1.005, 0.985 * mid);
        cross_t = std::min(v[cut] * 0.995, 1.015 * mid);
    }
    int classify(double t) const { return t < same_t ? 0 : (t <= cross_t ? 1 : 2); }
};

typedef unsigned u32x4 __attribute__((ext_vector_type(4)));

__global__ __launch_bounds__(256) void zone_probe_kernel(u32x4* w0, u32x4* w1) {
    extern __shared__ unsigned char occupancy_pad[];
    const int tid = threadIdx.x;
#pragma unroll 1
    for (int k = 0; k < 2; ++k) {
        u32x4* dst = (k ? w1 : w0) + (size_t)blockIdx.x * 1323;
#pragma unroll
        for (int j = 0; j < 5; ++j) dst[tid + 256 * j] = (u32x4)(0u);
        if (tid < 43) dst[tid + 1280] = (u32x4)(0u);
    }
}

__global__ __launch_bounds__(256) void store_probe_linear_kernel(u32x4* out, size_t nvec) {
    const size_t i = (size_t)blockIdx.x * 256 + threadIdx.x;
    if (i < nvec) out[i] = (u32x4)(0u);
}
__global__ __launch_bounds__(256) void store_probe_frames_kernel(u32x4* out, int n) {
    extern __shared__ unsigned char occupancy_pad[];
    const int tid = threadIdx.x;
    for (int f = blockIdx.x; f < n; f += gridDim.x) {
        u32x4* dst = out + (size_t)f * 1323;
#pragma unroll
        for (int j = 0; j < 5; ++j) dst[tid + 256 * j] = (u32x4)(0u);
        if (tid < 43) dst[tid + 1280] = (u32x4)(0u);
    }
}

__global__ __launch_bounds__(256) void store_probe_lines_kernel(u32x4* out, int n) {
    extern __shared__ unsigned char occupancy_pad[];
    const int tid = threadIdx.x;
    const size_t end = (size_t)n * 1323;
    for (int f = blockIdx.x; f < n; f += gridDim.x) {
        size_t v0 = ((size_t)f * 1323 + 7) & ~(size_t)7, v1 = ((size_t)(f + 1) * 1323 + 7) & ~(size_t)7;
        if (f == 0) v0 = 0;
        if (v1 > end) v1 = end;
#pragma unroll
        for (int j = 0; j < 6; ++j) {
            const size_t v = v0 + tid + 256 * j;
            if (v < v1) out[v] = (u32x4)(0u);
        }
    }
}
__device__ __forceinline__ int xcd_grouped_frame(int v) { return (v & ~63) | ((v & 7) << 3) | ((v >> 3) & 7); }
__global__ __launch_bounds__(256) void store_probe_frames_xcd_kernel(u32x4* out, int n) {
    extern __shared__ unsigned char occupancy_pad[];
    const int tid = threadIdx.x;
    for (int v = blockIdx.x; v < n; v += gridDim.x) {
        const int f = (v | 63) < n ? xcd_grouped_frame(v) : v;
        u32x4* dst = out + (size_t)f * 1323;
#pragma unroll
        for (int j = 0; j < 5; ++j) dst[tid + 256 * j] = (u32x4)(0u);
        if (tid < 43) dst[tid + 1280] = (u32x4)(0u);
    }
}
__global__ __launch_bounds__(256) void store_probe_octets_kernel(u32x4* out, int n) {
    extern __shared__ unsigned char occupancy_pad[];
    const int tid = threadIdx.x;
    const size_t end = (size_t)n * 1323;
    for (int g = blockIdx.x; g * 8 < n; g += gridDim.x) {
#pragma unroll 1
        for (int k = 0; k < 8 && g * 8 + k < n; ++k) {
            const size_t f = (size_t)g * 8 + k;
            size_t v0 = (f * 1323 + 3) & ~(size_t)3, v1 = ((f + 1) * 1323 + 3) & ~(size_t)3;
            if (v1 > end) v1 = end;
#pragma unroll
            for (int j = 0; j < 6; ++j) {
                const size_t v = v0 + tid + 256 * j;
                if (v < v1) out[v] = (u32x4)(0u);
            }
        }
    }
}
__global__ __launch_bounds__(256) void store_probe_frame_per_wg_kernel(u32x4* out) {
    const int tid = threadIdx.x;
    u32x4* dst = out + (size_t)blockIdx.x * 1323;
#pragma unroll
    for (int j = 0; j < 5; ++j) dst[tid + 256 * j] = (u32x4)(0u);
    if (tid < 43) dst[tid + 1280] = (u32x4)(0u);
}

__global__ __launch_bounds__(256) void store_probe_frames_pairs_kernel(u32x4* out, int n, int wave_quarters) {
    extern __shared__ unsigned char occupancy_pad[];
    const int tid = threadIdx.x;
    for (int f = blockIdx.x; f < n; f += gridDim.x) {
        u32x4* dst = out + (size_t)f * 1323;
        if (!wave_quarters) {
#pragma unroll
            for (int j = 0; j < 3; ++j) {
                const int v = 2 * tid + 512 * j;
                if (v < 1323) dst[v] = (u32x4)(0u);
                if (v + 1 < 1323) dst[v + 1] = (u32x4)(0u);
            }
        } else {
            const int w = tid >> 6, lane = tid & 63, lo = w * 332, hi = w == 3 ? 1323 : lo + 332;
#pragma unroll
            for (int j = 0; j < 3; ++j) {
                const int v = lo + 2 * lane + 128 * j;
                if (v < hi) dst[v] = (u32x4)(0u);
                if (v + 1 < hi) dst[v + 1] = (u32x4)(0u);
            }
        }
    }
}

inline void va_free(void* va, size_t bytes) {
    static const bool reuse = lab_env("MEMGYM_OBS_REUSE_VA") && atoi(lab_env("MEMGYM_OBS_REUSE_VA")) != 0;
    if (reuse) (void)hipMemAddressFree(va, bytes);
}

__global__ void verify_fill_kernel(u32x4* p, size_t nvec, unsigned salt) {
    for (size_t i = (size_t)blockIdx.x * blockDim.x + threadIdx.x; i < nvec; i += (size_t)gridDim.x * blockDim.x) {
        const unsigned h = (unsigned)i * 2654435761u + salt;
        p[i] = (u32x4){h, h ^ 0x9E3779B9u, (unsigned)(i >> 32) + salt, ~h};
    }
}
__global__ void verify_check_kernel(const u32x4* p, size_t nvec, unsigned salt, unsigned long long* bad) {
    unsigned long long mine = 0;
    for (size_t i = (size_t)blockIdx.x * blockDim.x + threadIdx.x; i < nvec; i += (size_t)gridDim.x * blockDim.x) {
        const unsigned h = (unsigned)i * 2654435761u + salt;
        const u32x4 v = p[i];
        mine += (v.x != h) | (v.y != (h ^ 0x9E3779B9u)) | (v.z != (unsigned)(i >> 32) + salt) | (v.w != ~h);
    }
    if (mine) atomicAdd(bad, mine);
}

struct Piece {
    hipMemGenericAllocationHandle_t h = nullptr;
    size_t bytes = 0;
};

struct Mapping {
    size_t va_bytes = 0;
    void* base = nullptr;
    std::vector<std::pair<size_t, Piece>> pieces;
    std::vector<int> piece_class;
    bool plain = false;
    int device = 0;
};

std::mutex g_mu;
std::map<void*, Mapping> g_live;

hipMemAllocationProp prop_for(int device) {
    hipMemAllocationProp p = {};
    p.type = hipMemAllocationTypePinned;
    p.location.type = hipMemLocationTypeDevice;
    p.location.id = device;
    return p;
}

size_t g_va_reserved = 0;
hipError_t va_reserve(void** va, size_t bytes) {
    const hipError_t e = hipMemAddressReserve(va, bytes, 2 * MiB, nullptr, 0);
    if (e == hipSuccess) g_va_reserved += bytes;
    return e;
}

bool create_piece(int device, size_t bytes, Piece* out, bool exportable = false) {
    static const bool no_vmm = lab_env("MEMGYM_OBS_NO_VMM") && atoi(lab_env("MEMGYM_OBS_NO_VMM")) != 0;
    if (no_vmm) return false;
    hipMemAllocationProp p = prop_for(device);
    if (exportable) p.requestedHandleType = hipMemHandleTypePosixFileDescriptor;
    hipMemGenericAllocationHandle_t h;
    if (hipMemCreate(&h, bytes, &p, 0) != hipSuccess) {
        (void)hipGetLastError();
        return false;
    }
    out->h = h;
    out->bytes = bytes;
    return true;
}

void release_piece(Piece& p) {
    if (p.h) (void)hipMemRelease(p.h);
    p.h = nullptr;
}

void map_at(void* va, const Piece& p, int device) {
    MG_HIP(hipMemMap(va, p.bytes, 0, p.h, 0));
    static const std::vector<int> all = [] {
        int n = 0;
        if (hipGetDeviceCount(&n) != hipSuccess) n = 1;
        std::vector<int> v(n);
        for (int i = 0; i < n; ++i) v[i] = i;
        return v;
    }();
    hipMemAccessDesc acc = {};
    acc.location.type = hipMemLocationTypeDevice;
    acc.location.id = device;
    acc.flags = hipMemAccessFlagsProtReadWrite;
    MG_HIP(hipMemSetAccess(va, p.bytes, &acc, 1));
    for (int d : all) {
        if (d == device) continue;
        int can = 0;
        if (hipDeviceCanAccessPeer(&can, d, device) != hipSuccess || !can) {
            (void)hipGetLastError();
            continue;
        }
        acc.location.id = d;
        if (hipMemSetAccess(va, p.bytes, &acc, 1) != hipSuccess) (void)hipGetLastError();
    }
}

struct Cand {
    Piece piece;
    void* va = nullptr;
    double tbps = 0;
    bool make(int device, bool exportable = false) {
        if (!create_piece(device, PIECE, &piece, exportable)) return false;
        if (va_reserve(&va, PIECE) != hipSuccess) {
            release_piece(piece);
            return false;
        }
        map_at(va, piece, device);
        return true;
    }
    void unmap() {
        if (va) {
            (void)hipMemUnmap(va, PIECE);
            va_free(va, PIECE);
            va = nullptr;
        }
    }
    void drop() {
        unmap();
        release_piece(piece);
    }
};

unsigned long long verify_range(void* p, size_t bytes, unsigned salt) {
    unsigned long long* bad = nullptr;
    MG_HIP(hipMalloc((void**)&bad, sizeof *bad));
    MG_HIP(hipMemset(bad, 0, sizeof *bad));
    const size_t nvec = bytes / 16;
    hipLaunchKernelGGL(verify_fill_kernel, dim3(4096), dim3(256), 0, 0, (u32x4*)p, nvec, salt);
    MG_HIP(hipDeviceSynchronize());
    hipLaunchKernelGGL(verify_check_kernel, dim3(4096), dim3(256), 0, 0, (const u32x4*)p, nvec, salt, bad);
    unsigned long long h = 0;
    MG_HIP(hipMemcpy(&h, bad, sizeof h, hipMemcpyDeviceToHost));
    (void)hipFree(bad);
    return h;
}

double probe_tbps(void* a, void* b) {
    hipEvent_t e0, e1;
    MG_HIP(hipEventCreate(&e0));
    MG_HIP(hipEventCreate(&e1));
    float best = 1e30f;
    for (int r = 0; r < 4; ++r) {
        MG_HIP(hipEventRecord(e0, 0));
        hipLaunchKernelGGL(zone_probe_kernel, dim3(PROBE_GRID), dim3(256), 22528, 0, (u32x4*)a, (u32x4*)b);
        MG_HIP(hipEventRecord(e1, 0));
        MG_HIP(hipEventSynchronize(e1));
        float ms = 0;
        MG_HIP(hipEventElapsedTime(&ms, e0, e1));
        if (r > 0) best = std::min(best, ms);
    }
    (void)hipEventDestroy(e0);
    (void)hipEventDestroy(e1);
    return 2.0 * PROBE_GRID * 21168.0 / (best * 1e-3) / 1e12;
}

}

struct ZoneCache {
    std::map<int, std::vector<Piece>> pool;
    size_t pooled = 0;
    int next_id = 0;
    Calib calib;
};
constexpr size_t POOL_CAP = 10;
std::map<int, ZoneCache> g_zones;

void pool_put(ZoneCache& Z, int group, Piece p) {
    if (group >= 0 && Z.pooled < POOL_CAP) {
        Z.pool[group].push_back(p);
        Z.pooled++;
    } else {
        release_piece(p);
    }
}

struct Group {
    int id = -1;
    std::vector<Cand> pcs;
};

namespace {
double g_search_ms = 1500.0;
}

extern "C" {

int mg_obs_set_search_ms(double ms) {
    if (!(ms >= 0)) {
        mg::set_error("mg_obs_set_search_ms: need a bound >= 0");
        return -1;
    }
    std::lock_guard<std::mutex> lk(g_mu);
    g_search_ms = ms;
    return 0;
}

int mg_store_probe(void* buf, size_t n_frames, int pattern, void* stream_) {
    hipStream_t stream = (hipStream_t)stream_;
    if (!buf || n_frames == 0 || n_frames > (1u << 30) || pattern < 0 || pattern > 7) {
        mg::set_error("mg_store_probe: bad arguments");
        return -1;
    }
    if (pattern == 0) {
        const size_t nvec = n_frames * 1323;
        hipLaunchKernelGGL(store_probe_linear_kernel, dim3((unsigned)((nvec + 255) / 256)), dim3(256), 0, stream, (u32x4*)buf, nvec);
    } else if (pattern == 1) {
        const int grid = (int)std::min<size_t>(n_frames, PROBE_GRID);
        hipLaunchKernelGGL(store_probe_frames_kernel, dim3(grid), dim3(256), 22528, stream, (u32x4*)buf, (int)n_frames);
    } else if (pattern == 4) {
        const int grid = (int)std::min<size_t>(n_frames, PROBE_GRID);
        hipLaunchKernelGGL(store_probe_lines_kernel, dim3(grid), dim3(256), 22528, stream, (u32x4*)buf, (int)n_frames);
    } else if (pattern == 6) {
        const int grid = (int)std::min<size_t>(n_frames, PROBE_GRID);
        hipLaunchKernelGGL(store_probe_frames_xcd_kernel, dim3(grid), dim3(256), 22528, stream, (u32x4*)buf, (int)n_frames);
    } else if (pattern == 7) {
        const int grid = (int)std::min<size_t>((n_frames + 7) / 8, PROBE_GRID);
        hipLaunchKernelGGL(store_probe_octets_kernel, dim3(grid), dim3(256), 22528, stream, (u32x4*)buf, (int)n_frames);
    } else if (pattern == 5) {
        hipLaunchKernelGGL(store_probe_frame_per_wg_kernel, dim3((unsigned)n_frames), dim3(256), 0, stream, (u32x4*)buf);
    } else {
        const int grid = (int)std::min<size_t>(n_frames, PROBE_GRID);
        hipLaunchKernelGGL(store_probe_frames_pairs_kernel, dim3(grid), dim3(256), 22528, stream, (u32x4*)buf, (int)n_frames, pattern == 3 ? 1 : 0);
    }
    if (hipGetLastError() != hipSuccess) {
        mg::set_error("mg_store_probe: launch failed");
        return -1;
    }
    return 0;
}

static void plan_zones(size_t k, size_t lead, size_t window, size_t G, std::vector<size_t>& want, std::vector<size_t>& count) {
    want.assign(k, 0);
    count.assign(G, 0);
    size_t prev_w = (size_t)-1, j = 0;
    for (size_t p = 0; p < k; ++p) {
        const size_t centre = p * PIECE + PIECE / 2, w = centre > lead ? (centre - lead) / window : 0;
        j = w == prev_w ? j + 1 : 0;
        prev_w = w;
        want[p] = G == 2 ? (w + j) % 2 : p % G;
        ++count[want[p]];
    }
}
static size_t range_lead(size_t k, size_t bytes) { return ((k * PIECE - bytes) / 2) & ~(size_t)(2 * MiB - 1); }

int mg_obs_plan(size_t bytes, size_t frame_bytes, int zones, size_t* piece_bytes, size_t* lead_bytes, int* zone_of_piece, int max_pieces) {
    if (bytes == 0 || zones < 2 || zones > 3) {
        mg::set_error("mg_obs_plan: bad arguments");
        return -1;
    }
    const size_t k = (bytes + PIECE - 1) / PIECE;
    std::vector<size_t> want, count;
    plan_zones(k, range_lead(k, bytes), (frame_bytes ? frame_bytes : (size_t)mg::FRAME_BYTES) * (size_t)PROBE_GRID, (size_t)zones, want, count);
    if (piece_bytes) *piece_bytes = PIECE;
    if (lead_bytes) *lead_bytes = range_lead(k, bytes);
    for (size_t p = 0; p < k && (int)p < max_pieces; ++p)
        if (zone_of_piece) zone_of_piece[p] = (int)want[p];
    return (int)k;
}

int mg_obs_alloc(int device, size_t bytes, size_t search_budget_bytes, void** out, mg_obs_alloc_info* info) {
    return mg_obs_alloc_for(device, bytes, (size_t)mg::FRAME_BYTES, search_budget_bytes, out, info);
}

int mg_obs_alloc_for(int device, size_t bytes, size_t frame_bytes, size_t search_budget_bytes, void** out, mg_obs_alloc_info* info) {
    mg_obs_alloc_info I = {};
    try {
        if (!out || bytes == 0) {
            mg::set_error("mg_obs_alloc: bad arguments");
            return -1;
        }
        int prev = 0;
        MG_HIP(hipGetDevice(&prev));
        MG_HIP(hipSetDevice(device));
        struct Restore {
            int d;
            ~Restore() { (void)hipSetDevice(d); }
        } restore{prev};
        const auto t0 = std::chrono::steady_clock::now();
        const bool debug = lab_env("MEMGYM_OBS_DEBUG") != nullptr;
        *out = nullptr;
        size_t free_b = 0, total_b = 0;
        MG_HIP(hipMemGetInfo(&free_b, &total_b));
        if (search_budget_bytes == MG_OBS_SEARCH_DEFAULT) search_budget_bytes = std::min<size_t>(free_b / 2, 128 * GiB);
        const size_t k = (bytes + PIECE - 1) / PIECE;
        auto plain = [&](int zones) {
            void* p = nullptr;
            MG_HIP(hipMalloc(&p, bytes));
            Mapping m;
            m.plain = true;
            m.device = device;
            std::lock_guard<std::mutex> lk(g_mu);
            g_live[p] = m;
            *out = p;
            I.zones = zones;
            I.search_ms = std::chrono::duration<double, std::milli>(std::chrono::steady_clock::now() - t0).count();
            if (info) *info = I;
        };
        std::unique_lock<std::mutex> lock(g_mu);
        ZoneCache& Z = g_zones[device];
        if (k < 2 || (Z.pooled < k && (search_budget_bytes < PIECE || free_b < (k + 4) * PIECE))) {
            lock.unlock();
            plain(0);
            return 0;
        }
        const size_t half = (k + 1) / 2, loose_cap = k - std::max<size_t>(1, k / 4);
        std::vector<Group> groups;
        for (auto& kv : Z.pool) {
            if (kv.second.empty()) continue;
            Group g;
            g.id = kv.first;
            for (auto& p : kv.second) {
                Cand c;
                c.piece = p;
                g.pcs.push_back(c);
            }
            groups.push_back(g);
        }
        Z.pool.clear();
        Z.pooled = 0;
        auto usable = [&](size_t cap) {
            size_t u = 0;
            for (auto& g : groups) u += std::min(g.pcs.size(), cap);
            return u;
        };
        auto ref_va = [&](Group& g) {
            Cand& r = g.pcs[0];
            if (!r.va) {
                if (va_reserve(&r.va, PIECE) != hipSuccess) throw std::runtime_error("mg_obs_alloc: hipMemAddressReserve failed");
                map_at(r.va, r.piece, device);
            }
            return r.va;
        };
        std::vector<Cand> unclear;
        std::vector<Piece> spacers;
        size_t walked = 0;
        std::vector<std::pair<double, int>> decided;
        bool restarted = false;
        int tries_after_good = 0;
        bool exportable = false;
        auto give_back = [&] {
            for (auto& g : groups)
                for (auto& c : g.pcs) {
                    c.unmap();
                    pool_put(Z, g.id, c.piece);
                }
            groups.clear();
            for (auto& c : unclear) c.drop();
            unclear.clear();
            for (auto& sp : spacers) release_piece(sp);
            spacers.clear();
        };
        try {
            const double max_ms = g_search_ms;
            auto elapsed_ms = [&] { return std::chrono::duration<double, std::milli>(std::chrono::steady_clock::now() - t0).count(); };
            double step_max_ms = 0, release_ms_each = 0;
            auto held = [&] {
                size_t h = spacers.size() + unclear.size();
                for (auto& g : groups) h += g.pcs.size();
                return h;
            };
            auto out_of_time = [&] { return elapsed_ms() + step_max_ms + (double)held() * release_ms_each >= max_ms; };
            while ((usable(half) < k || groups.size() < 2) && walked <= search_budget_bytes && !out_of_time()) {
                const double step_t0 = elapsed_ms();
                struct StepClock {
                    double t0, *mx;
                    std::chrono::steady_clock::time_point base;
                    ~StepClock() {
                        const double now = std::chrono::duration<double, std::milli>(std::chrono::steady_clock::now() - base).count();
                        *mx = std::max(*mx, now - t0);
                    }
                } step_clock{step_t0, &step_max_ms, t0};
                Cand c;
                if (!c.make(device, exportable)) break;
                int home = -1;
                bool odd = false;
                for (size_t j = 0; j < groups.size() && home < 0; ++j) {
                    c.tbps = probe_tbps(ref_va(groups[j]), c.va);
                    Z.calib.observe(c.tbps);
                    const int cls = Z.calib.classify(c.tbps);
                    decided.push_back({c.tbps, cls});
                    if (cls == 0) {
                        home = (int)j;
                        I.probe_same_tbps = std::max(I.probe_same_tbps, c.tbps);
                    } else if (cls == 1) {
                        odd = true;
                        break;
                    } else {
                        I.probe_cross_tbps = I.probe_cross_tbps == 0 ? c.tbps : std::min(I.probe_cross_tbps, c.tbps);
                    }
                }
                if (!restarted && Z.calib.relative) {
                    bool differs = false;
                    for (auto& d : decided) differs = differs || Z.calib.classify(d.first) != d.second;
                    if (differs) {
                        if (debug) fprintf(stderr, "mg_obs_alloc: thresholds now %.2f / %.2f TB/s (relative): starting over\n", Z.calib.same_t, Z.calib.cross_t);
                        restarted = true;
                        c.drop();
                        for (auto& g : groups)
                            for (auto& q : g.pcs) q.drop();
                        groups.clear();
                        for (auto& q : unclear) q.drop();
                        unclear.clear();
                        decided.clear();
                        I.probe_same_tbps = I.probe_cross_tbps = 0;
                        continue;
                    }
                }
                if (debug)
                    fprintf(stderr, "mg_obs_alloc: %5.1f GiB walked, %s piece: last probe %.2f TB/s -> %s\n", walked / (double)GiB,
                            exportable ? "exportable" : "ordinary", c.tbps, odd ? "unclear" : home >= 0 ? "known group" : "new group");
                bool useful = false;
                if (odd) {
                    unclear.push_back(c);
                } else if (home < 0) {
                    Group g;
                    g.id = Z.next_id++;
                    g.pcs.push_back(c);
                    groups.push_back(g);
                    useful = true;
                } else {
                    useful = groups[home].pcs.size() < half;
                    c.unmap();
                    groups[home].pcs.push_back(c);
                }
                if (useful) continue;
                walked += PIECE;
                const bool good_enough = groups.size() >= 2 && usable(loose_cap) >= k;
                const bool early = elapsed_ms() < 0.25 * max_ms;
                if (good_enough && ++tries_after_good > 6 && !early) break;
                exportable = !exportable;
                if (!exportable && (!good_enough || early)) {
                    const size_t before = spacers.size();
                    for (int f = 0; f < FILL_STEP && walked + PIECE <= search_budget_bytes && !out_of_time(); ++f) {
                        Piece sp;
                        const double c0 = elapsed_ms();
                        if (!create_piece(device, PIECE, &sp)) break;
                        if (release_ms_each == 0) {
                            const double r0 = elapsed_ms();
                            release_piece(sp);
                            release_ms_each = std::max(1e-3, elapsed_ms() - r0);
                            if (!create_piece(device, PIECE, &sp)) break;
                        }
                        step_max_ms = std::max(step_max_ms, elapsed_ms() - c0);
                        spacers.push_back(sp);
                        walked += PIECE;
                    }
                    if (spacers.size() == before) break;
                }
            }
        } catch (...) {
            give_back();
            throw;
        }
        I.searched_bytes = walked;
        I.zones = (int)std::min<size_t>(groups.size(), 3);
        if (groups.size() < 2 || usable(k) < k) {
            const bool one = groups.size() < 2;
            give_back();
            lock.unlock();
            if (debug) fprintf(stderr, "mg_obs_alloc: %s after %.1f GiB: plain allocation\n", one ? "one zone only" : "not enough pieces", walked / (double)GiB);
            plain(1);
            return 0;
        }
        const size_t cap = usable(half) >= k ? half : (usable(loose_cap) >= k ? loose_cap : k);
        std::sort(groups.begin(), groups.end(), [](const Group& x, const Group& y) { return x.pcs.size() > y.pcs.size(); });
        const size_t lead = range_lead(k, bytes);
        const size_t window = (frame_bytes ? frame_bytes : (size_t)mg::FRAME_BYTES) * (size_t)PROBE_GRID;
        std::vector<size_t> want, count;
        plan_zones(k, lead, window, 2, want, count);
        bool alternating = true;
        for (size_t p = 0; p < k; ++p) alternating = alternating && want[p] == p % 2;
        std::vector<std::pair<Piece, int>> order;
        if (alternating) {
            for (size_t round = 0; round < cap && order.size() < k; ++round)
                for (auto& g : groups)
                    if (round < g.pcs.size() && order.size() < k) {
                        g.pcs[round].unmap();
                        order.push_back({g.pcs[round].piece, g.id});
                        g.pcs[round].piece.h = nullptr;
                    }
        } else {
            size_t zones_used = 0;
            for (size_t G = 2; G <= std::min<size_t>(groups.size(), 3); ++G) {
                plan_zones(k, lead, window, G, want, count);
                zones_used = G;
                std::vector<size_t> need(count);
                std::sort(need.begin(), need.end(), [](size_t a, size_t b) { return a > b; });
                bool fits = true;
                for (size_t r = 0; r < G; ++r) fits = fits && need[r] <= std::min(groups[r].pcs.size(), cap);
                if (fits) break;
            }
            std::vector<size_t> by_count(zones_used), group_of(zones_used);
            for (size_t z = 0; z < zones_used; ++z) by_count[z] = z;
            std::stable_sort(by_count.begin(), by_count.end(), [&](size_t a, size_t b) { return count[a] > count[b]; });
            for (size_t r = 0; r < zones_used; ++r) group_of[by_count[r]] = r;
            std::vector<size_t> taken(groups.size(), 0);
            for (size_t p = 0; p < k; ++p) {
                size_t gi = group_of[want[p]];
                if (taken[gi] >= std::min(groups[gi].pcs.size(), cap)) {
                    size_t best = groups.size(), room = 0;
                    for (size_t g2 = 0; g2 < groups.size(); ++g2) {
                        const size_t lim = std::min(groups[g2].pcs.size(), cap), left = lim - std::min(taken[g2], lim);
                        if (left > room) {
                            room = left;
                            best = g2;
                        }
                    }
                    if (best == groups.size()) throw std::runtime_error("mg_obs_alloc: internal error (pieces ran out while assembling)");
                    gi = best;
                }
                Cand& c = groups[gi].pcs[taken[gi]++];
                c.unmap();
                order.push_back({c.piece, groups[gi].id});
                c.piece.h = nullptr;
            }
        }
        for (auto& g : groups) {
            std::vector<Cand> rest;
            for (auto& c : g.pcs)
                if (c.piece.h) rest.push_back(c);
            g.pcs.swap(rest);
        }
        give_back();
        void* va = nullptr;
        if (va_reserve(&va, k * PIECE) != hipSuccess) {
            for (auto& o : order) pool_put(Z, o.second, o.first);
            throw std::runtime_error("mg_obs_alloc: hipMemAddressReserve failed");
        }
        Mapping m;
        m.va_bytes = k * PIECE;
        m.device = device;
        for (size_t i = 0; i < k; ++i) {
            map_at((char*)va + i * PIECE, order[i].first, device);
            m.pieces.push_back({i * PIECE, order[i].first});
            m.piece_class.push_back(order[i].second);
        }
        if (const unsigned long long bad = verify_range(va, k * PIECE, 0x5EEDu)) {
            for (auto& op : m.pieces) {
                (void)hipMemUnmap((char*)va + op.first, op.second.bytes);
                (void)hipMemRelease(op.second.h);
            }
            throw std::runtime_error("mg_obs_alloc: " + std::to_string(bad) + " of " + std::to_string(k * PIECE / 16) +
                                     " vectors of the assembled range did not read back (stale translations?)");
        }
        m.base = va;
        void* user = (char*)va + lead;
        g_live[user] = m;
        *out = user;
        I.pieces = (int)k;
        I.piece_bytes = PIECE;
        I.search_ms = std::chrono::duration<double, std::milli>(std::chrono::steady_clock::now() - t0).count();
        if (debug) {
            std::string lay;
            for (auto& o : order) lay += (char)('A' + (o.second % 26));
            fprintf(stderr, "mg_obs_alloc: %zu pieces %s, %.1f GiB walked, %.0f ms, %zu spare pieces pooled\n", k, lay.c_str(),
                    walked / (double)GiB, I.search_ms, Z.pooled);
        }
        if (info) *info = I;
        return 0;
    } catch (const std::exception& e) {
        mg::set_error(e.what());
        return -1;
    }
}

int mg_obs_debug_stats(size_t* live_buffers, size_t* pooled_pieces, size_t* reserved_va_bytes) {
    std::lock_guard<std::mutex> lk(g_mu);
    if (live_buffers) *live_buffers = g_live.size();
    size_t pooled = 0;
    for (auto& z : g_zones) pooled += z.second.pooled;
    if (pooled_pieces) *pooled_pieces = pooled;
    if (reserved_va_bytes) *reserved_va_bytes = g_va_reserved;
    return 0;
}

int mg_obs_free(void* p) {
    if (!p) return 0;
    Mapping m;
    {
        std::lock_guard<std::mutex> lk(g_mu);
        auto it = g_live.find(p);
        if (it == g_live.end()) {
            mg::set_error("mg_obs_free: not a pointer returned by mg_obs_alloc");
            return -1;
        }
        m = it->second;
        g_live.erase(it);
    }
    int prev = 0;
    (void)hipGetDevice(&prev);
    (void)hipSetDevice(m.device);
    struct Restore {
        int d;
        ~Restore() { (void)hipSetDevice(d); }
    } restore{prev};
    if (m.plain) return hipFree(p) == hipSuccess ? 0 : -1;
    (void)hipDeviceSynchronize();
    std::lock_guard<std::mutex> lk(g_mu);
    ZoneCache& Z = g_zones[m.device];
    for (size_t i = 0; i < m.pieces.size(); ++i) {
        (void)hipMemUnmap((char*)m.base + m.pieces[i].first, m.pieces[i].second.bytes);
        pool_put(Z, i < m.piece_class.size() ? m.piece_class[i] : -1, m.pieces[i].second);
    }
    va_free(m.base, m.va_bytes);
    return 0;
}

}
```

### endless-memory-gym_amd/memory_gym_amd/__init__.py

```python
from .reset_params import DEFAULTS, process_reset_params
from .vec_env import ENV_IDS, MemoryGymEnv, VecMemoryGym, alloc_obs_buffer
from .vector import GymnasiumVectorEnv
from . import envs



def make(env_id, num_envs=None, device=None, render_mode=None, obs_format="u8_xyc", final_observation=False, obs_buffer=None,
         obs_placement=None, ground_truth64=False, on_capacity="raise", capacity=None):
    if num_envs is None:
        if env_id not in envs.CLASSES:
            raise ValueError("unknown env id %r" % (env_id,))
        return envs.CLASSES[env_id](render_mode=render_mode, device=device, capacity=capacity)
    return VecMemoryGym(env_id, num_envs=num_envs, device=device, render_mode=render_mode, obs_format=obs_format,
                        final_observation=final_observation, obs_buffer=obs_buffer, obs_placement=obs_placement,
                        ground_truth64=ground_truth64, on_capacity=on_capacity, capacity=capacity)


def _register_with_gymnasium():
    try:
        from gymnasium.envs.registration import register
    except Exception:
        return
    for env_id, entry_point in envs.ENTRY_POINTS.items():
        try:
            register(id=env_id, entry_point=entry_point)
        except Exception:
            pass


_register_with_gymnasium()
```

### endless-memory-gym_amd/memory_gym_amd/_native.py

```python
import ctypes as C
import os

import torch

PKG_ROOT = os.path.dirname(os.path.dirname(os.path.abspath(__file__)))
LIB_PATH = os.environ.get("MEMGYM_HIP_LIB", os.path.join(PKG_ROOT, "lib", "libmemgym_hip.so"))

MG_INFO_SLOTS = 8
MG_MAX_OPTION_SETS = 8


class InfoBuffers(C.Structure):
    _fields_ = [("struct_size", C.c_size_t), ("ep_reward_dev", C.c_void_p), ("ep_length_dev", C.c_void_p), ("aux_dev", C.c_void_p * MG_INFO_SLOTS),
                ("final_obs_dev", C.c_void_p), ("reward64_dev", C.c_void_p), ("gt64_dev", C.c_void_p), ("capacity_dev", C.c_void_p)]


class SingleIO(C.Structure):
    _fields_ = [("struct_size", C.c_size_t), ("obs", C.c_void_p), ("vec", C.c_void_p), ("reward", C.c_void_p), ("done", C.c_void_p),
                ("gt", C.c_void_p), ("ep_reward", C.c_void_p), ("ep_length", C.c_void_p), ("aux", C.c_void_p * MG_INFO_SLOTS)]


class ObsAllocInfo(C.Structure):
    _fields_ = [("zones", C.c_int), ("pieces", C.c_int), ("piece_bytes", C.c_size_t), ("searched_bytes", C.c_size_t),
                ("probe_same_tbps", C.c_double), ("probe_cross_tbps", C.c_double), ("search_ms", C.c_double)]


MG_OBS_SEARCH_DEFAULT = (1 << 64) - 1


def _load():
    if not os.path.exists(LIB_PATH):
        raise ImportError(
            "memory_gym_amd: native library %s not found. Build it with `python __graft_entry__.py` "
            "(hipcc --offload-arch=gfx950). There is no fallback path." % LIB_PATH)
    L = C.CDLL(LIB_PATH)
    L.mg_last_error.restype = C.c_char_p
    L.mg_create.argtypes = [C.c_char_p, C.c_int32, C.c_int, C.POINTER(C.c_void_p)]
    L.mg_destroy.argtypes = [C.c_void_p]
    L.mg_destroy.restype = None
    for f in ("mg_num_envs", "mg_action_dim", "mg_gt_dim"):
        getattr(L, f).argtypes = [C.c_void_p]
        getattr(L, f).restype = C.c_int32
    L.mg_info_name.argtypes = [C.c_void_p, C.c_int]
    L.mg_info_name.restype = C.c_char_p
    L.mg_set_option.argtypes = [C.c_void_p, C.c_char_p, C.POINTER(C.c_double), C.c_int]
    L.mg_vec_dim.argtypes = [C.c_void_p]
    L.mg_vec_dim.restype = C.c_int32
    L.mg_bind_vector_obs.argtypes = [C.c_void_p, C.c_void_p]
    L.mg_set_obs_format.argtypes = [C.c_void_p, C.c_int]
    L.mg_obs_bytes.argtypes = [C.c_void_p]
    L.mg_obs_bytes.restype = C.c_size_t
    L.mg_reset.argtypes = [C.c_void_p, C.c_void_p, C.c_void_p, C.c_void_p, C.c_void_p, C.c_void_p]
    L.mg_step.argtypes = [C.c_void_p, C.c_void_p, C.c_void_p, C.c_void_p, C.c_void_p, C.c_void_p, C.POINTER(InfoBuffers),
                          C.c_int, C.c_void_p]
    L.mg_render.argtypes = [C.c_void_p, C.c_void_p, C.c_void_p]
    L.mg_render_debug.argtypes = [C.c_void_p, C.c_void_p, C.c_void_p]
    L.mg_state_size.argtypes = [C.c_void_p]
    L.mg_state_size.restype = C.c_size_t
    L.mg_get_state.argtypes = [C.c_void_p, C.c_void_p, C.c_size_t]
    L.mg_set_state.argtypes = [C.c_void_p, C.c_void_p, C.c_size_t]
    L.mg_set_profiling.argtypes = [C.c_void_p, C.c_int]
    L.mg_get_profile.argtypes = [C.c_void_p, C.c_int, C.POINTER(C.c_double), C.POINTER(C.c_int64)]
    L.mg_poll_errors.argtypes = [C.c_void_p, C.POINTER(C.c_int)]
    L.mg_peek_errors.argtypes = [C.c_void_p, C.POINTER(C.c_int)]
    L.mg_obs_alloc.argtypes = [C.c_int, C.c_size_t, C.c_size_t, C.POINTER(C.c_void_p), C.POINTER(ObsAllocInfo)]
    if hasattr(L, "mg_obs_alloc_for"):
        L.mg_obs_alloc_for.argtypes = [C.c_int, C.c_size_t, C.c_size_t, C.c_size_t, C.POINTER(C.c_void_p), C.POINTER(ObsAllocInfo)]
        L.mg_obs_plan.argtypes = [C.c_size_t, C.c_size_t, C.c_int, C.POINTER(C.c_size_t), C.POINTER(C.c_size_t), C.POINTER(C.c_int), C.c_int]
    L.mg_obs_free.argtypes = [C.c_void_p]
    L.mg_obs_debug_stats.argtypes = [C.POINTER(C.c_size_t), C.POINTER(C.c_size_t), C.POINTER(C.c_size_t)]
    if hasattr(L, "mg_single_open"):
        L.mg_ground_truth64.argtypes = [C.c_void_p, C.c_void_p, C.c_void_p]
        L.mg_single_open.argtypes = [C.c_void_p, C.POINTER(SingleIO)]
        L.mg_single_reset.argtypes = [C.c_void_p, C.c_int64, C.c_int, C.c_void_p]
        L.mg_single_step.argtypes = [C.c_void_p, C.c_int32, C.c_int32, C.c_void_p]
    if hasattr(L, "mg_obs_set_search_ms"):
        L.mg_obs_set_search_ms.argtypes = [C.c_double]
        L.mg_store_probe.argtypes = [C.c_void_p, C.c_size_t, C.c_int, C.c_void_p]
    L.mg_enable_peer_access.argtypes = [C.c_int, C.c_int]
    L.mg_debug_rng.argtypes = [C.c_void_p, C.c_int32, C.c_void_p]
    if hasattr(L, "mg_set_option_set"):
        L.mg_set_option_set.argtypes = [C.c_void_p, C.c_int, C.c_char_p, C.POINTER(C.c_double), C.c_int]
        L.mg_bind_option_sets.argtypes = [C.c_void_p, C.c_void_p]
    L.mg_set_capacity.argtypes = [C.c_void_p, C.c_char_p, C.c_int64]
    L.mg_capacity.argtypes = [C.c_void_p, C.c_char_p]
    L.mg_capacity.restype = C.c_int64
    if hasattr(L, "mg_debug_counter"):
        L.mg_debug_counter.argtypes = [C.c_void_p, C.c_char_p, C.POINTER(C.c_int64)]
    return L


LIB = _load()


def last_error():
    return (LIB.mg_last_error() or b"").decode()


def check(rc, what):
    if rc == -3:
        raise NotImplementedError("%s: %s" % (what, last_error()))
    if rc != 0:
        raise RuntimeError("%s failed (%d): %s" % (what, rc, last_error()))
```

### endless-memory-gym_amd/memory_gym_amd/vec_env.py

```python
import ctypes as C
import os
import weakref

import numpy as np
import torch

from . import _native
from .reset_params import DEFAULTS, calc_max_episode_steps, process_reset_params

ENV_IDS = list(DEFAULTS.keys())


class _Space:
    def __init__(self, kind, **kw):
        self.kind = kind
        self.__dict__.update(kw)

    def __repr__(self):
        return "%s(%s)" % (self.kind, ", ".join("%s=%r" % kv for kv in self.__dict__.items() if kv[0] != "kind"))


def _spaces(action_dim, gt_dim, vec_dim=0):
    try:
        from gymnasium import spaces
        act = spaces.Discrete(4) if action_dim == 1 else spaces.MultiDiscrete([3, 3])
        obs = spaces.Box(low=0, high=255, shape=[84, 84, 3], dtype=np.uint8)
        if vec_dim:
            obs = spaces.Dict({"visual_observation": obs,
                               "vector_observation": spaces.Box(low=np.zeros(vec_dim, np.float32), high=np.ones(vec_dim, np.float32),
                                                                shape=(vec_dim,), dtype=np.float32)})
        gt = None if gt_dim == 0 else spaces.Box(low=np.zeros(gt_dim, np.float32), high=np.ones(gt_dim, np.float32),
                                                  shape=(gt_dim,), dtype=np.float32)
    except Exception:
        act = _Space("Discrete", n=4) if action_dim == 1 else _Space("MultiDiscrete", nvec=[3, 3])
        obs = _Space("Box", low=0, high=255, shape=[84, 84, 3], dtype=np.uint8)
        if vec_dim:
            obs = _Space("Dict", spaces={"visual_observation": obs, "vector_observation": _Space(
                "Box", low=0.0, high=1.0, shape=(vec_dim,), dtype=np.float32)})
        gt = None if gt_dim == 0 else _Space("Box", low=0.0, high=1.0, shape=(gt_dim,), dtype=np.float32)
    return act, obs, gt


_BALANCED = weakref.WeakSet()


def is_balanced_buffer(tensor):
    p = tensor.data_ptr()
    return any(o.ptr is not None and o.ptr <= p < o.ptr + o.nbytes for o in _BALANCED)


class _ObsMemory:

    def __init__(self, ptr, shape, typestr, info):
        self.ptr, self.info = ptr, info
        self.nbytes = int(np.prod(shape))
        _BALANCED.add(self)
        self.__cuda_array_interface__ = {"shape": tuple(shape), "typestr": typestr, "data": (ptr, False), "version": 2, "strides": None}

    def __del__(self):
        try:
            if self.ptr:
                _native.LIB.mg_obs_free(C.c_void_p(self.ptr))
                self.ptr = None
        except Exception:
            pass


def alloc_obs_buffer(shape, dtype, device, search_budget_bytes=None, frame_bytes=None):
    device = torch.device(device)
    elem = torch.empty((), dtype=dtype).element_size()
    nbytes = int(np.prod(shape)) * elem
    if search_budget_bytes is None:
        e = os.environ.get("MEMGYM_OBS_SEARCH_GB")
        search_budget_bytes = _native.MG_OBS_SEARCH_DEFAULT if e is None else int(float(e) * (1 << 30))
    ms = os.environ.get("MEMGYM_OBS_SEARCH_MS")
    if ms is not None and hasattr(_native.LIB, "mg_obs_set_search_ms"):
        _native.check(_native.LIB.mg_obs_set_search_ms(float(ms)), "mg_obs_set_search_ms")
    ptr, info = C.c_void_p(), _native.ObsAllocInfo()
    with torch.cuda.device(device):
        torch.cuda.current_stream().synchronize()
        if frame_bytes is None:
            frame_bytes = int(np.prod(shape[1:])) * elem if len(shape) > 1 else 84 * 84 * 3
        lab = os.environ.get("MEMGYM_OBS_FRAME_BYTES")
        if lab:
            frame_bytes = int(lab)
        if hasattr(_native.LIB, "mg_obs_alloc_for"):
            _native.check(_native.LIB.mg_obs_alloc_for(device.index or 0, nbytes, C.c_size_t(frame_bytes), C.c_size_t(search_budget_bytes), C.byref(ptr),
                                                       C.byref(info)), "mg_obs_alloc_for")
        else:
            _native.check(_native.LIB.mg_obs_alloc(device.index or 0, nbytes, C.c_size_t(search_budget_bytes), C.byref(ptr), C.byref(info)), "mg_obs_alloc")
    owner = _ObsMemory(ptr.value, (nbytes,), "|u1", {k: getattr(info, k) for k, _ in info._fields_})
    t = torch.as_tensor(owner, device=device).view(dtype).view(tuple(shape))
    return t, owner.info


class VecMemoryGym:
    metadata = {"render_modes": ["rgb_array", "debug_rgb_array"], "render_fps": 25}

    OBS_FORMATS = {"u8_xyc": (0, torch.uint8, (84, 84, 3)), "f32_chw": (1, torch.float32, (3, 84, 84)),
                   "f16_chw": (2, torch.float16, (3, 84, 84)), "bf16_chw": (3, torch.bfloat16, (3, 84, 84))}

    def __init__(self, env_id, num_envs=1, device=None, render_mode=None, obs_format="u8_xyc", final_observation=False,
                 obs_buffer=None, obs_placement=None, ground_truth64=False, on_capacity="raise", capacity=None):
        if env_id not in DEFAULTS:
            raise ValueError("unknown env id %r" % (env_id,))
        if obs_format not in self.OBS_FORMATS:
            raise ValueError("obs_format must be one of %s" % sorted(self.OBS_FORMATS))
        if not torch.cuda.is_available():
            raise RuntimeError("memory_gym_amd needs a ROCm GPU (MI355X); no CPU fallback exists")
        self.env_id = env_id
        self.num_envs = int(num_envs)
        self.device = torch.device("cuda", torch.cuda.current_device() if device is None else
                                   (device if isinstance(device, int) else torch.device(device).index or 0))
        self.render_mode = render_mode
        h = C.c_void_p()
        _native.check(_native.LIB.mg_create(env_id.encode(), self.num_envs, self.device.index, C.byref(h)), "mg_create")
        self._h = h
        self.capacity = {}
        for what, value in (capacity or {}).items():
            with torch.cuda.device(self.device):
                rc = _native.LIB.mg_set_capacity(h, what.encode(), int(value))
            if rc != 0:
                raise ValueError("capacity[%r] = %r: %s" % (what, value, _native.last_error()))
            self.capacity[what] = int(value)
        self.action_dim = _native.LIB.mg_action_dim(h)
        self.gt_dim = _native.LIB.mg_gt_dim(h)
        self.vec_dim = _native.LIB.mg_vec_dim(h)
        self.has_ground_truth_info = self.gt_dim > 0
        self.action_space, self.observation_space, self.ground_truth_space = _spaces(self.action_dim, self.gt_dim, self.vec_dim)
        N, dev = self.num_envs, self.device
        self.obs_format = obs_format
        code, dt, shape = self.OBS_FORMATS[obs_format]
        _native.check(_native.LIB.mg_set_obs_format(h, code), "mg_set_obs_format")
        assert _native.LIB.mg_obs_bytes(h) == 84 * 84 * 3 * torch.empty((), dtype=dt).element_size()
        self.obs_placement_info = None
        if obs_placement is None:
            obs_placement = os.environ.get("MEMGYM_OBS_PLACEMENT", "balanced")
        if obs_placement not in ("balanced", "plain"):
            raise ValueError("obs_placement must be 'balanced' or 'plain'")
        if obs_buffer is None:
            nbytes = N * 84 * 84 * 3 * torch.empty((), dtype=dt).element_size()
            self.obs = None
            if obs_placement == "balanced" and nbytes > (304 << 20):
                try:
                    self.obs, self.obs_placement_info = alloc_obs_buffer((N,) + shape, dt, dev)
                except RuntimeError as e:
                    import warnings
                    warnings.warn("memory_gym_amd: balanced observation buffer not available (%s); using a plain allocation" % (e,))
            if self.obs is None:
                self.obs = torch.empty((N,) + shape, dtype=dt, device=dev)
        else:
            if tuple(obs_buffer.shape) != (N,) + shape or obs_buffer.dtype != dt or not obs_buffer.is_cuda or not obs_buffer.is_contiguous():
                raise ValueError("obs_buffer must be a contiguous CUDA tensor of shape %s and dtype %s" % ((N,) + shape, dt))
            self.obs = obs_buffer
        self.final_obs = torch.zeros((N,) + shape, dtype=dt, device=dev) if final_observation else None
        self.vector_obs = None
        if self.vec_dim:
            self.vector_obs = torch.zeros((N, self.vec_dim), dtype=torch.float32, device=dev)
            _native.check(_native.LIB.mg_bind_vector_obs(h, self.vector_obs.data_ptr()), "mg_bind_vector_obs")
        self.reward = torch.zeros(N, dtype=torch.float32, device=dev)
        self.reward64 = torch.zeros(N, dtype=torch.float64, device=dev)
        self.done_u8 = torch.zeros(N, dtype=torch.uint8, device=dev)
        self.gt = torch.zeros((N, max(self.gt_dim, 1)), dtype=torch.float32, device=dev)
        self.gt64 = torch.zeros((N, max(self.gt_dim, 1)), dtype=torch.float64, device=dev) if (ground_truth64 and self.gt_dim) else None
        self.ep_reward = torch.zeros(N, dtype=torch.float64, device=dev)
        self.ep_length = torch.zeros(N, dtype=torch.int32, device=dev)
        self.info_names = []
        for k in range(_native.MG_INFO_SLOTS):
            nm = _native.LIB.mg_info_name(h, k)
            if nm is None:
                break
            self.info_names.append(nm.decode())
        self.aux = [torch.zeros(N, dtype=torch.float32, device=dev) for _ in self.info_names]
        self._info = _native.InfoBuffers()
        self._info.struct_size = C.sizeof(_native.InfoBuffers)
        self._err = C.c_int(0)
        self._info.ep_reward_dev = self.ep_reward.data_ptr()
        self._info.ep_length_dev = self.ep_length.data_ptr()
        for k, t in enumerate(self.aux):
            self._info.aux_dev[k] = t.data_ptr()
        self._info.final_obs_dev = self.final_obs.data_ptr() if self.final_obs is not None else None
        self._info.reward64_dev = self.reward64.data_ptr()
        self._info.gt64_dev = self.gt64.data_ptr() if self.gt64 is not None else None
        if on_capacity not in ("raise", "truncate"):
            raise ValueError("on_capacity must be 'raise' or 'truncate'")
        self.on_capacity = on_capacity
        self.capacity_u8 = torch.zeros(N, dtype=torch.uint8, device=dev) if on_capacity == "truncate" else None
        self._info.capacity_dev = self.capacity_u8.data_ptr() if self.capacity_u8 is not None else None
        self._tolerated = self.CAPACITY_BITS if on_capacity == "truncate" else 0
        self.reset_params = process_reset_params(env_id, None)
        self._applied = dict(DEFAULTS[env_id])
        self._set_params = [self._applied]
        self._set_of = None
        self.max_episode_steps = None
        self.autoreset = True
        self._seeded = False
        self._swapped = False
        self._truncated = self.capacity_u8.view(torch.bool) if self.capacity_u8 is not None else torch.zeros(N, dtype=torch.bool, device=dev)
        self._n_actions = self.num_envs * self.action_dim
        self._p_err = C.byref(self._err)
        self._bind_step()

    def _stream(self):
        return C.c_void_p(self._raw_stream())

    def _raw_stream(self):
        try:
            return torch._C._cuda_getCurrentRawStream(self.device.index)
        except AttributeError:
            return torch.cuda.current_stream(self.device).cuda_stream

    def _bind_step(self):
        self._p_reward = self.reward.data_ptr()
        self._p_done = self.done_u8.data_ptr()
        self._p_gt = self.gt.data_ptr() if self.gt_dim else None
        self._p_info = C.byref(self._info)
        self._done_bool = self.done_u8.view(torch.bool)
        info = {"done_mask": self._done_bool, "reward": self.ep_reward, "length": self.ep_length}
        for nm, t in zip(self.info_names, self.aux):
            info[nm] = t
        if self.gt_dim:
            info["ground_truth"] = self.gt if self.gt64 is None else self.gt64
        if self.capacity_u8 is not None:
            info["capacity_exceeded"] = self._truncated
        self._info_dict = info

    def _write_set(self, set_id, params):
        have = self._set_params[set_id]
        for k, v in params.items():
            if k in have and have[k] == v:
                continue
            vals = [float(x) for x in v] if isinstance(v, (list, tuple, np.ndarray)) else [float(v)]
            arr = (C.c_double * len(vals))(*vals)
            if set_id == 0:
                rc = _native.LIB.mg_set_option(self._h, k.encode(), arr, len(vals))
            else:
                rc = _native.LIB.mg_set_option_set(self._h, set_id, k.encode(), arr, len(vals))
            if rc == -2:
                raise AssertionError("Provided reset parameter (" + str(k) + ") is not valid. Check spelling.")
            if rc == -4:
                raise AssertionError(_native.last_error())
            if rc != 0:
                raise NotImplementedError("reset parameter %s=%r%s: %s" % (k, v, "" if set_id == 0 else " for a subset of the instances", _native.last_error()))
            have[k] = v

    def _apply_options_masked(self, options, mask):
        if options is None:
            return
        params = process_reset_params(self.env_id, options)
        k = next((j for j, p in enumerate(self._set_params) if p == params), None)
        if k == 0 and self._set_of is None:
            return
        if k is None:
            used = set([0])
            if self._set_of is not None:
                used |= set(torch.unique(self._set_of).cpu().tolist())
            free = [j for j in range(1, _native.MG_MAX_OPTION_SETS) if j not in used]
            if not free:
                raise NotImplementedError("more than %d different option sets alive in one handle" % _native.MG_MAX_OPTION_SETS)
            k = free[0]
            while len(self._set_params) <= k:
                self._set_params.append({})
            self._set_params[k] = {}
            try:
                self._write_set(k, params)
            except Exception:
                self._set_params[k] = {}
                raise
        if self._set_of is None:
            self._set_of = torch.zeros(self.num_envs, dtype=torch.int32, device=self.device)
            _native.check(_native.LIB.mg_bind_option_sets(self._h, self._set_of.data_ptr()), "mg_bind_option_sets")
        self._set_of[mask.to(device=self.device, dtype=torch.bool)] = k

    def _apply_options(self, options):
        params = process_reset_params(self.env_id, options)
        self._write_set(0, params)
        if self._set_of is not None:
            _native.check(_native.LIB.mg_bind_option_sets(self._h, None), "mg_bind_option_sets")
            self._set_of = None
        del self._set_params[1:]
        self.reset_params = params
        if self.env_id in ("MortarMayhemB-Grid-v0", "MortarMayhemB-v0"):
            self.max_episode_steps = calc_max_episode_steps(
                max(params["command_count"]), 0, 0, max(params["explosion_delay"]), max(params["explosion_duration"]))
        elif self.env_id in ("MortarMayhem-Grid-v0", "MortarMayhem-v0"):
            self.max_episode_steps = calc_max_episode_steps(
                max(params["command_count"]), max(params["command_show_duration"]), max(params["command_show_delay"]),
                max(params["explosion_delay"]), max(params["explosion_duration"]))
        else:
            self.max_episode_steps = params.get("max_steps", None)

    def _seed_tensor(self, seed):
        if seed is None:
            if self._seeded:
                return None
            seed = np.random.SeedSequence().generate_state(self.num_envs, np.uint64) >> np.uint64(1)
            seed = seed.astype(np.int64)
        if isinstance(seed, torch.Tensor):
            s = seed.to(device=self.device, dtype=torch.int64)
        elif np.isscalar(seed):
            s = torch.arange(self.num_envs, device=self.device, dtype=torch.int64) + int(seed)
        else:
            s = torch.as_tensor(np.asarray(seed, dtype=np.int64), device=self.device)
        assert s.numel() == self.num_envs
        return s.contiguous()

    def reset(self, seed=None, return_info=True, options=None, mask=None):
        with torch.cuda.device(self.device):
            if mask is not None and seed is None and not self._seeded:
                raise RuntimeError("a masked reset(seed=None) needs an earlier full reset: the other instances have no RNG stream yet")
            if mask is None:
                self._apply_options(options)
            else:
                self._apply_options_masked(options, mask)
            s = self._seed_tensor(seed)
            m = None if mask is None else mask.to(device=self.device, dtype=torch.uint8).contiguous()
            if m is not None and self._swapped:
                _native.check(_native.LIB.mg_render(self._h, self.obs.data_ptr(), self._stream()), "mg_render")
            self._swapped = False
            _native.check(_native.LIB.mg_reset(self._h, None if s is None else s.data_ptr(),
                                               None if m is None else m.data_ptr(), self.obs.data_ptr(),
                                               self.gt.data_ptr() if self.gt_dim else None, self._stream()), "mg_reset")
            if self.gt64 is not None:
                _native.check(_native.LIB.mg_ground_truth64(self._h, self.gt64.data_ptr(), self._stream()), "mg_ground_truth64")
            self._seeded = True
        info = {"ground_truth": self.gt if self.gt64 is None else self.gt64} if self.gt_dim else {}
        return self._obs(), info

    def step(self, actions):
        a = actions
        if not (isinstance(a, torch.Tensor) and a.dtype == torch.int32 and a.device == self.device and a.is_contiguous()):
            a = a if isinstance(a, torch.Tensor) else torch.as_tensor(np.asarray(a))
            a = a.to(device=self.device, dtype=torch.int32).contiguous()
        assert a.numel() == self._n_actions, "actions must have shape [N] or [N, 2]"
        if torch.cuda.current_device() != self.device.index:
            with torch.cuda.device(self.device):
                self._launch_step(a)
        else:
            self._launch_step(a)
        self._swapped = False
        _native.LIB.mg_peek_errors(self._h, self._p_err)
        if self._err.value & ~self._tolerated:
            self.check_errors()
        info = dict(self._info_dict)
        if self.final_obs is not None and self.autoreset:
            info["final_observation"] = self.final_obs
        return self._obs(), self.reward, self._done_bool, self._truncated, info

    def _launch_step(self, a):
        rc = _native.LIB.mg_step(self._h, a.data_ptr(), self.obs.data_ptr(), self._p_reward, self._p_done, self._p_gt, self._p_info,
                                 1 if self.autoreset else 0, self._raw_stream())
        if rc != 0:
            _native.check(rc, "mg_step")

    def new_obs_buffer(self):
        if self.obs_placement_info is not None:
            try:
                t, _ = alloc_obs_buffer(tuple(self.obs.shape), self.obs.dtype, self.device)
                return t
            except RuntimeError:
                pass
        return torch.empty_like(self.obs)

    def use_obs_buffer(self, tensor):
        if tuple(tensor.shape) != tuple(self.obs.shape) or tensor.dtype != self.obs.dtype or tensor.device != self.obs.device or not tensor.is_contiguous():
            raise ValueError("use_obs_buffer: need a contiguous tensor like env.obs")
        self.obs = tensor
        self._swapped = True
        self._bind_step()

    def use_step_buffers(self, reward, done_u8):
        for t, dt in ((reward, torch.float32), (done_u8, torch.uint8)):
            if tuple(t.shape) != (self.num_envs,) or t.dtype != dt or t.device != self.device or not t.is_contiguous():
                raise ValueError("use_step_buffers: need contiguous float32 [N] / uint8 [N] tensors on the handle's device")
        if reward.data_ptr() % 4:
            raise ValueError("use_step_buffers: the reward tensor must be 4-byte aligned")
        self.reward, self.done_u8 = reward, done_u8
        self._bind_step()

    def _obs(self):
        if self.vector_obs is None:
            return self.obs
        return {"visual_observation": self.obs, "vector_observation": self.vector_obs}

    def render(self):
        if self.render_mode == "debug_rgb_array":
            return self.render_debug()
        if self.obs_format != "u8_xyc":
            return (self.obs.permute(0, 2, 3, 1).float() * 255.0).round().to(torch.uint8)
        return self.obs.permute(0, 2, 1, 3)

    def render_debug(self):
        out = torch.empty((self.num_envs, 336, 336, 3), dtype=torch.uint8, device=self.device)
        with torch.cuda.device(self.device):
            _native.check(_native.LIB.mg_render_debug(self._h, out.data_ptr(), self._stream()), "mg_render_debug")
        return out

    def state_dict(self):
        n = _native.LIB.mg_state_size(self._h)
        buf = np.empty(n, np.uint8)
        with torch.cuda.device(self.device):
            _native.check(_native.LIB.mg_get_state(self._h, buf.ctypes.data, n), "mg_get_state")
        sd = {"env_id": self.env_id, "num_envs": self.num_envs, "blob": buf, "options": dict(self._applied), "seeded": self._seeded,
              "capacity": dict(self.capacity)}
        if self._set_of is not None:
            sd["option_sets"] = [dict(p) for p in self._set_params]
            sd["set_of"] = self._set_of.cpu().numpy()
        return sd

    def load_state_dict(self, sd):
        assert sd["env_id"] == self.env_id and sd["num_envs"] == self.num_envs
        if sd.get("capacity", {}) != self.capacity:
            raise ValueError("the checkpoint was taken with capacity=%r, this handle was made with %r" % (sd.get("capacity", {}), self.capacity))
        with torch.cuda.device(self.device):
            opts = sd.get("options")
            if opts is not None and any(self._applied.get(k) != v for k, v in opts.items()):
                self.reset(seed=0, options={k: v for k, v in opts.items() if k in DEFAULTS[self.env_id]})
                _native.LIB.mg_poll_errors(self._h, C.byref(C.c_int()))
            if sd.get("option_sets") is not None:
                for k, p in enumerate(sd["option_sets"]):
                    while len(self._set_params) <= k:
                        self._set_params.append({})
                    if k > 0 and p:
                        self._set_params[k] = {}
                        self._write_set(k, process_reset_params(self.env_id, {kk: vv for kk, vv in p.items() if kk in DEFAULTS[self.env_id]}))
                if self._set_of is None:
                    self._set_of = torch.zeros(self.num_envs, dtype=torch.int32, device=self.device)
                    _native.check(_native.LIB.mg_bind_option_sets(self._h, self._set_of.data_ptr()), "mg_bind_option_sets")
                self._set_of.copy_(torch.as_tensor(np.asarray(sd["set_of"], dtype=np.int32), device=self.device))
            elif self._set_of is not None:
                _native.check(_native.LIB.mg_bind_option_sets(self._h, None), "mg_bind_option_sets")
                self._set_of = None
                del self._set_params[1:]
            buf = np.ascontiguousarray(sd["blob"], dtype=np.uint8)
            _native.check(_native.LIB.mg_set_state(self._h, buf.ctypes.data, buf.size), "mg_set_state")
            self._seeded = bool(sd.get("seeded", True))

    def set_profiling(self, every):
        _native.check(_native.LIB.mg_set_profiling(self._h, int(every)), "mg_set_profiling")

    def get_profile(self, kind):
        ms, n = C.c_double(), C.c_int64()
        _native.check(_native.LIB.mg_get_profile(self._h, kind, C.byref(ms), C.byref(n)), "mg_get_profile")
        return ms.value, n.value

    CAPACITY_BITS = 1 | 4 | 8 | 32

    ERROR_BITS = {1: "more than 16 live spotlights in one instance (raise spawn_interval / spot speeds or lower initial_spawns)",
                  2: "path generation found no valid path (pygame_assets.py:723-724 raises here too)",
                  4: "endless path longer than 128 segments", 8: "more than 128 distinct fall-off cells",
                  16: "past-path window wider than 16 columns",
                  32: "Endless Mortar Mayhem command list reached its 512-entry capacity (the episode was ended)",
                  64: "a deferred-reset queue overflowed (a previous fused launch did not drain it)",
                  256: "use_exit=False for an instance that never had an exit (the reference raises AttributeError at this reset)"}

    def check_errors(self):
        f = C.c_int()
        _native.check(_native.LIB.mg_poll_errors(self._h, C.byref(f)), "mg_poll_errors")
        self.capacity_events = getattr(self, "capacity_events", 0) | (f.value & self._tolerated)
        f.value &= ~self._tolerated
        if f.value:
            what = "; ".join(m for b, m in self.ERROR_BITS.items() if f.value & b)
            hint = " (make(..., on_capacity='truncate') reports such instances as truncated instead of raising)" if f.value & self.CAPACITY_BITS else ""
            raise RuntimeError("memory_gym_amd: device error flags 0x%x: %s -- the frames of the affected instances are "
                               "no longer the reference's (include/memgym.h: mg_poll_errors)%s" % (f.value, what, hint))

    def rng_words(self, i):
        w = np.zeros(6, np.uint64)
        _native.check(_native.LIB.mg_debug_rng(self._h, int(i), w.ctypes.data), "mg_debug_rng")
        return w

    def debug_counter(self, name):
        v = C.c_int64()
        _native.check(_native.LIB.mg_debug_counter(self._h, name.encode(), C.byref(v)), "mg_debug_counter")
        return v.value

    def close(self):
        if getattr(self, "_h", None):
            _native.LIB.mg_destroy(self._h)
            self._h = None

    def __del__(self):
        try:
            self.close()
        except Exception:
            pass


try:
    import gymnasium as _gym
    _EnvBase = _gym.Env
except Exception:
    _gym = None
    _EnvBase = object


class MemoryGymEnv(_EnvBase):

    metadata = {"render_modes": ["rgb_array", "debug_rgb_array"], "render_fps": 25}
    spec = None
    env_id = None

    def __init__(self, env_id=None, device=None, render_mode=None, capacity=None):
        env_id = env_id or self.env_id
        self.vec = VecMemoryGym(env_id, 1, device, render_mode, capacity=capacity)
        self.vec.autoreset = False
        self.action_space = self.vec.action_space
        self.observation_space = self.vec.observation_space
        self.has_ground_truth_info = self.vec.has_ground_truth_info
        if self.has_ground_truth_info:
            self.ground_truth_space = self.vec.ground_truth_space
        self.render_mode = render_mode
        self._np_random = None
        io = _native.SingleIO()
        io.struct_size = C.sizeof(_native.SingleIO)
        with torch.cuda.device(self.vec.device):
            _native.check(_native.LIB.mg_single_open(self.vec._h, C.byref(io)), "mg_single_open")
        self._io = io

        def view(ptr, ctype, shape):
            return np.ctypeslib.as_array(C.cast(ptr, C.POINTER(ctype)), shape=shape)
        self._obs_host = view(io.obs, C.c_uint8, (84, 84, 3))
        self._vec_host = view(io.vec, C.c_float, (self.vec.vec_dim,)) if self.vec.vec_dim else None
        self._reward_host = view(io.reward, C.c_double, (1,))
        self._done_host = view(io.done, C.c_uint8, (1,))
        self._gt_host = view(io.gt, C.c_double, (max(self.vec.gt_dim, 1),))
        self._ep_reward_host = view(io.ep_reward, C.c_double, (1,))
        self._ep_length_host = view(io.ep_length, C.c_int32, (1,))
        self._aux_host = [view(io.aux[k], C.c_float, (1,)) for k in range(len(self.vec.info_names))]
        self._two_actions = self.vec.action_dim == 2
        self._raw_stream = self.vec._raw_stream
        self._step_fn, self._h, self._errword = _native.LIB.mg_single_step, self.vec._h, self.vec._err
        if self.vec.vector_obs is not None:
            self.vec.vector_obs_stale = True
        self._peek = _native.LIB.mg_peek_errors

    @property
    def unwrapped(self):
        return self

    @property
    def np_random(self):
        if self._np_random is None:
            self._np_random = np.random.Generator(np.random.PCG64(np.random.SeedSequence()))
        return self._np_random

    @np_random.setter
    def np_random(self, value):
        self._np_random = value

    def _observation(self):
        o = self._obs_host.copy()
        if self._vec_host is not None:
            o = {"visual_observation": o, "vector_observation": self._vec_host.copy()}
        return o

    @property
    def max_episode_steps(self):
        return self.vec.max_episode_steps

    def reset(self, seed=None, return_info=True, options=None):
        if seed is not None:
            self._np_random = np.random.Generator(np.random.PCG64(np.random.SeedSequence(int(seed))))
        v = self.vec
        with torch.cuda.device(v.device):
            v._apply_options(options)
            if seed is None and not v._seeded:
                seed = int(np.random.SeedSequence().generate_state(1, np.uint64)[0] >> np.uint64(1))
            _native.check(_native.LIB.mg_single_reset(self._h, 0 if seed is None else int(seed), 0 if seed is None else 1, C.c_void_p(self._raw_stream())), "mg_single_reset")
            v._seeded = True
        out = {}
        if v.gt_dim:
            out["ground_truth"] = self._gt_host[:v.gt_dim].copy()
        return self._observation(), out

    def step(self, action):
        if self._two_actions:
            a0, a1 = int(action[0]), int(action[1])
        else:
            a0 = a1 = int(action)
        rc = self._step_fn(self._h, a0, a1, self._raw_stream())
        if rc != 0:
            if rc < 0:
                _native.check(rc, "mg_single_step")
            if rc & ~self.vec._tolerated:
                self.vec.check_errors()
        r, d = float(self._reward_host[0]), bool(self._done_host[0])
        out = {}
        if d:
            out["reward"] = float(self._ep_reward_host[0])
            out["length"] = int(self._ep_length_host[0])
            for nm, a in zip(self.vec.info_names, self._aux_host):
                out[nm] = float(a[0])
        if self.vec.gt_dim:
            out["ground_truth"] = self._gt_host[:self.vec.gt_dim].copy()
        return self._observation(), r, d, False, out

    def render(self):
        if self.render_mode == "debug_rgb_array":
            return self.vec.render_debug()[0].cpu().numpy()
        return self._obs_host.transpose(1, 0, 2).copy()

    def state_dict(self):
        return self.vec.state_dict()

    def load_state_dict(self, sd):
        self.vec.load_state_dict(sd)

    def close(self):
        self.vec.close()
```

### include/memgym.h

```cpp
#ifndef MEMGYM_H
#define MEMGYM_H
#include <stddef.h>
#include <stdint.h>

#ifdef __cplusplus
extern "C" {
#endif

typedef struct mg_env mg_env;

#define MG_OBS_DIM 84
#define MG_OBS_BYTES (84 * 84 * 3)
#define MG_INFO_SLOTS 8

typedef struct mg_info_buffers {
    size_t struct_size;
    double* ep_reward_dev;
    int32_t* ep_length_dev;
    float* aux_dev[MG_INFO_SLOTS];
    void* final_obs_dev;
    double* reward64_dev;
    double* gt64_dev;
    uint8_t* capacity_dev;
} mg_info_buffers;

int mg_create(const char* env_id, int32_t num_envs, int device, mg_env** out);
void mg_destroy(mg_env* env);
const char* mg_last_error(void);

int32_t mg_num_envs(const mg_env* env);
int32_t mg_action_dim(const mg_env* env);
int32_t mg_gt_dim(const mg_env* env);
int32_t mg_vec_dim(const mg_env* env);
int mg_bind_vector_obs(mg_env* env, float* vec_dev);
const char* mg_info_name(const mg_env* env, int k);

int mg_set_option(mg_env* env, const char* key, const double* values, int n);

#define MG_MAX_OPTION_SETS 8
int mg_set_option_set(mg_env* env, int set_id, const char* key, const double* values, int n);
int mg_bind_option_sets(mg_env* env, const int32_t* set_of_dev);

int mg_set_capacity(mg_env* env, const char* what, int64_t value);
int64_t mg_capacity(mg_env* env, const char* what);

#define MG_OBS_U8_XYC 0
#define MG_OBS_F32_CYX 1
#define MG_OBS_F16_CYX 2
#define MG_OBS_BF16_CYX 3
int mg_set_obs_format(mg_env* env, int format);
size_t mg_obs_bytes(const mg_env* env);

int mg_reset(mg_env* env, const int64_t* seeds_dev, const uint8_t* mask_dev, void* obs_dev, float* gt_dev,
             void* stream);

int mg_render(mg_env* env, void* obs_dev, void* stream);

int mg_render_debug(mg_env* env, uint8_t* rgb_dev, void* stream);

int mg_step(mg_env* env, const int32_t* actions_dev, void* obs_dev, float* reward_dev, uint8_t* done_dev,
            float* gt_dev, const mg_info_buffers* info, int autoreset, void* stream);

int mg_ground_truth64(mg_env* env, double* gt64_dev, void* stream);

typedef struct mg_single_io {
    size_t struct_size;
    void* obs;
    float* vec;
    double* reward;
    uint8_t* done;
    double* gt;
    double* ep_reward;
    int32_t* ep_length;
    float* aux[MG_INFO_SLOTS];
} mg_single_io;
int mg_single_open(mg_env* env, mg_single_io* io);
int mg_single_reset(mg_env* env, int64_t seed, int has_seed, void* stream);
int mg_single_step(mg_env* env, int32_t a0, int32_t a1, void* stream);

#define MG_STATE_VERSION 8u
size_t mg_state_size(const mg_env* env);
int mg_get_state(mg_env* env, void* host_buf, size_t size);
int mg_set_state(mg_env* env, const void* host_buf, size_t size);

int mg_set_profiling(mg_env* env, int on);
int mg_get_profile(mg_env* env, int kind, double* total_ms, int64_t* launches);

int mg_poll_errors(mg_env* env, int* flags);

int mg_peek_errors(mg_env* env, int* flags);

typedef struct mg_obs_alloc_info {
    int zones;
    int pieces;
    size_t piece_bytes;
    size_t searched_bytes;
    double probe_same_tbps;
    double probe_cross_tbps;
    double search_ms;
} mg_obs_alloc_info;
#define MG_OBS_SEARCH_DEFAULT ((size_t)-1)
int mg_obs_alloc(int device, size_t bytes, size_t search_budget_bytes, void** out_dev, mg_obs_alloc_info* info);
int mg_obs_alloc_for(int device, size_t bytes, size_t frame_bytes, size_t search_budget_bytes, void** out_dev, mg_obs_alloc_info* info);
int mg_obs_plan(size_t bytes, size_t frame_bytes, int zones, size_t* piece_bytes, size_t* lead_bytes, int* zone_of_piece, int max_pieces);
int mg_obs_free(void* obs_dev);
int mg_obs_set_search_ms(double ms);
int mg_store_probe(void* obs_dev, size_t n_frames, int pattern, void* stream);
int mg_obs_debug_stats(size_t* live_buffers, size_t* pooled_pieces, size_t* reserved_va_bytes);

int mg_enable_peer_access(int device, int peer_device);

int mg_debug_counter(mg_env* env, const char* name, int64_t* value);

int mg_debug_rng(mg_env* env, int32_t i, uint64_t* out);

#ifdef __cplusplus
}
#endif
#endif
```

Before: 292.3 million env steps/s.

## Rasterize Mortar frames incrementally by redrawing only dirty regions since last step

Keeps a per-env copy of the last drawn descriptor. The fused step+raster kernel compares it with the new descriptor, skips envs whose frame is unchanged, and limits writes to the dirty boxes of the template, sprite and glyph. Frame polling is batched per wavefront: one lane per env loads descriptors, and readlane then serves each frame. Host-side write tracking, Python tensor-version checks and invalidation hooks keep the retained obs buffer valid, at the cost of extra bookkeeping and a correctness risk if outside code writes the buffer.

```diff
diff --git a/endless-memory-gym_amd/csrc/mg_api.hip b/endless-memory-gym_amd/csrc/mg_api.hip
--- a/endless-memory-gym_amd/csrc/mg_api.hip
+++ b/endless-memory-gym_amd/csrc/mg_api.hip
@@ -3,6 +3,7 @@
 #include <cstddef>
 #include <map>
 #include <mutex>
+#include <vector>
 
 #include "mg_family.hpp"
 #include "mg_lab.hpp"
@@ -11,6 +12,54 @@
 namespace mg {
 static thread_local std::string g_last_error;
 void set_error(const std::string& msg) { g_last_error = msg; }
+
+namespace {
+struct ObsWrite {
+    const void* writer;
+    uintptr_t lo, hi;
+    uint64_t seq;
+};
+constexpr size_t OBS_WRITES_MAX = 256;
+std::mutex g_obs_mu;
+std::vector<ObsWrite> g_obs_writes;
+uint64_t g_obs_seq = 0, g_obs_lost = 0;
+}
+uint64_t obs_write_note(const void* writer, const void* p, size_t bytes) {
+    std::lock_guard<std::mutex> lk(g_obs_mu);
+    const uintptr_t lo = (uintptr_t)p, hi = lo + bytes;
+    const uint64_t seq = ++g_obs_seq;
+    for (ObsWrite& w : g_obs_writes)
+        if (w.writer == writer && w.lo == lo && w.hi == hi) {
+            w.seq = seq;
+            return seq;
+        }
+    if (g_obs_writes.size() >= OBS_WRITES_MAX) {
+        auto oldest = std::min_element(g_obs_writes.begin(), g_obs_writes.end(), [](const ObsWrite& a, const ObsWrite& b) { return a.seq < b.seq; });
+        g_obs_lost = std::max(g_obs_lost, oldest->seq);
+        g_obs_writes.erase(oldest);
+    }
+    g_obs_writes.push_back({writer, lo, hi, seq});
+    return seq;
+}
+void obs_write_forget(const void* writer) {
+    std::lock_guard<std::mutex> lk(g_obs_mu);
+    for (size_t k = 0; k < g_obs_writes.size();)
+        if (g_obs_writes[k].writer == writer) {
+            g_obs_lost = std::max(g_obs_lost, g_obs_writes[k].seq);
+            g_obs_writes[k] = g_obs_writes.back();
+            g_obs_writes.pop_back();
+        } else {
+            ++k;
+        }
+}
+bool obs_written_by_other(const void* reader, const void* p, size_t bytes, uint64_t since) {
+    std::lock_guard<std::mutex> lk(g_obs_mu);
+    if (g_obs_lost > since) return true;
+    const uintptr_t lo = (uintptr_t)p, hi = lo + bytes;
+    for (const ObsWrite& w : g_obs_writes)
+        if (w.writer != reader && w.seq > since && w.lo < hi && lo < w.hi) return true;
+    return false;
+}
 }
 
 struct mg_env {
@@ -169,6 +218,7 @@
     (void)hipGetDevice(&prev);
     (void)hipSetDevice(env->device);
     (void)hipDeviceSynchronize();
+    mg::obs_write_forget(env->fam);
     destroy_family(env);
     delete env;
     if (prev >= 0) (void)hipSetDevice(prev);
@@ -213,6 +263,7 @@
         if (!what) throw mg::OptionError{-3, "mg_set_capacity: NULL"};
         if (env->started) throw std::runtime_error("mg_set_capacity: before the first mg_reset / mg_set_state");
         env->fam->set_capacity(what, value);
+        env->fam->invalidate_frames();
     });
 }
 int64_t mg_capacity(mg_env* env, const char* what) {
@@ -229,6 +280,7 @@
         if (format != MG_OBS_U8_XYC && format != MG_OBS_F32_CYX && format != MG_OBS_F16_CYX && format != MG_OBS_BF16_CYX)
             throw mg::OptionError{-3, "mg_set_obs_format: unknown format"};
         env->obs_format = env->fam->obs_format = format;
+        env->fam->invalidate_frames();
     });
 }
 
@@ -240,6 +292,8 @@
 int mg_reset(mg_env* env, const int64_t* seeds_dev, const uint8_t* mask_dev, void* obs_dev, float* gt_dev, void* stream) {
     return guarded(env, [&] {
         if (!obs_dev) throw std::runtime_error("mg_reset: obs_dev is NULL");
+        env->fam->invalidate_frames();
+        mg::obs_write_note(env->fam, obs_dev, (size_t)env->num_envs * mg_obs_bytes(env));
         env->fam->reset(seeds_dev, mask_dev, obs_dev, gt_dev, (hipStream_t)stream);
         env->started = true;
     });
@@ -248,6 +302,7 @@
 int mg_render(mg_env* env, void* obs_dev, void* stream) {
     return guarded(env, [&] {
         if (!obs_dev) throw std::runtime_error("mg_render: obs_dev is NULL");
+        mg::obs_write_note(env->fam, obs_dev, (size_t)env->num_envs * mg_obs_bytes(env));
         env->fam->raster_only(obs_dev, nullptr, (hipStream_t)stream);
     });
 }
@@ -317,6 +372,12 @@
     });
 }
 
+}
+namespace {
+void step_call(mg_env* env, mg::Family* f, const int32_t* actions_dev, void* obs_dev, float* reward_dev, uint8_t* done_dev, float* gt_dev,
+               const mg_info_buffers& ib, int autoreset, hipStream_t st);
+}
+extern "C" {
 int mg_step(mg_env* env, const int32_t* actions_dev, void* obs_dev, float* reward_dev, uint8_t* done_dev, float* gt_dev,
             const mg_info_buffers* info, int autoreset, void* stream) {
     return guarded(env, [&] {
@@ -324,21 +385,46 @@
         hipStream_t st = (hipStream_t)stream;
         const mg_info_buffers ib = read_info(info);
         mg::Family* f = env->fam;
-        if (autoreset && ib.final_obs_dev && !(mg::sparse_masked_raster() && f->keeps_final_obs(st))) {
-            f->step(actions_dev, obs_dev, reward_dev, done_dev, gt_dev, &ib, 0, st);
-            if (mg::sparse_masked_raster()) {
-                const int n = env->num_envs, vec_per_row = (int)(mg_obs_bytes(env) / 16);
-                hipLaunchKernelGGL(copy_rows_kernel, dim3(std::min((n + COPY_CHUNK - 1) / COPY_CHUNK, 16384)), dim3(256), 0, st, done_dev, (const row_vec16*)obs_dev,
-                                   (row_vec16*)ib.final_obs_dev, n, vec_per_row);
-                MG_HIP(hipGetLastError());
-            } else f->raster_only(ib.final_obs_dev, done_dev, st);
-            f->reset(nullptr, done_dev, obs_dev, gt_dev, st);
-        } else {
-            f->step(actions_dev, obs_dev, reward_dev, done_dev, gt_dev, &ib, autoreset, st);
-        }
-        if (ib.gt64_dev) f->ground_truth64(ib.gt64_dev, st);
-    });
-}
+        try {
+            step_call(env, f, actions_dev, obs_dev, reward_dev, done_dev, gt_dev, ib, autoreset, st);
+        } catch (...) {
+            f->invalidate_frames();
+            throw;
+        }
+    });
+}
+
+int mg_invalidate_frames(mg_env* env) {
+    return guarded(env, [&] { env->fam->invalidate_frames(); });
+}
+
+int mg_set_incremental_frames(mg_env* env, int on) {
+    return guarded(env, [&] { env->fam->set_incremental_frames(on != 0); });
+}
+
+}
+namespace {
+void step_call(mg_env* env, mg::Family* f, const int32_t* actions_dev, void* obs_dev, float* reward_dev, uint8_t* done_dev, float* gt_dev,
+               const mg_info_buffers& ib, int autoreset, hipStream_t st) {
+    const size_t rows = (size_t)env->num_envs * mg_obs_bytes(env);
+    mg::obs_write_note(f, obs_dev, rows);
+    if (ib.final_obs_dev) mg::obs_write_note(f, ib.final_obs_dev, rows);
+    if (autoreset && ib.final_obs_dev && !(mg::sparse_masked_raster() && f->keeps_final_obs(st))) {
+        f->step(actions_dev, obs_dev, reward_dev, done_dev, gt_dev, &ib, 0, st);
+        if (mg::sparse_masked_raster()) {
+            const int n = env->num_envs, vec_per_row = (int)(mg_obs_bytes(env) / 16);
+            hipLaunchKernelGGL(copy_rows_kernel, dim3(std::min((n + COPY_CHUNK - 1) / COPY_CHUNK, 16384)), dim3(256), 0, st, done_dev, (const row_vec16*)obs_dev,
+                               (row_vec16*)ib.final_obs_dev, n, vec_per_row);
+            MG_HIP(hipGetLastError());
+        } else f->raster_only(ib.final_obs_dev, done_dev, st);
+        f->reset(nullptr, done_dev, obs_dev, gt_dev, st);
+    } else {
+        f->step(actions_dev, obs_dev, reward_dev, done_dev, gt_dev, &ib, autoreset, st);
+    }
+    if (ib.gt64_dev) f->ground_truth64(ib.gt64_dev, st);
+}
+}
+extern "C" {
 
 int mg_ground_truth64(mg_env* env, double* gt64_dev, void* stream) {
     return guarded(env, [&] {
@@ -415,6 +501,7 @@
         hipStream_t st = (hipStream_t)stream;
         *(int64_t*)(S.host + S.o_seed) = seed;
         mg::Family* f = env->fam;
+        f->invalidate_frames();
         f->reset(has_seed ? (const int64_t*)(S.dev + S.o_seed) : nullptr, nullptr, S.dev + S.o_obs, f->gt_dim() ? (float*)(S.dev + S.o_gt32) : nullptr, st);
         f->ground_truth64((double*)(S.dev + S.o_gt), st);
         env->started = true;
@@ -439,6 +526,7 @@
         for (int k = 0; k < MG_INFO_SLOTS; ++k) ib.aux_dev[k] = (float*)(S.dev + S.o_aux + 256 * k);
         ib.reward64_dev = (double*)(S.dev + S.o_reward);
         mg::Family* f = env->fam;
+        f->invalidate_frames();
         const bool armed = f->arm_done_flag((uint32_t*)(S.dev + S.o_flag), S.ticket + 1);
         if (armed) ++S.ticket;
         f->step((const int32_t*)(S.dev + S.o_action), S.dev + S.o_obs, (float*)(S.dev + S.o_reward32), (uint8_t*)(S.dev + S.o_done),
@@ -500,6 +588,7 @@
             p += b.second;
         }
         env->fam->on_state_loaded();
+        env->fam->invalidate_frames();
         env->started = true;
     });
 }
diff --git a/endless-memory-gym_amd/csrc/mg_family.hpp b/endless-memory-gym_amd/csrc/mg_family.hpp
--- a/endless-memory-gym_amd/csrc/mg_family.hpp
+++ b/endless-memory-gym_amd/csrc/mg_family.hpp
@@ -211,7 +211,13 @@
     virtual int poll_errors() { return 0; }
     virtual int peek_errors() { return 0; }
     virtual bool debug_counter(const std::string& , int64_t* ) { return false; }
-};
+    virtual void invalidate_frames() {}
+    virtual void set_incremental_frames(bool ) {}
+};
+
+uint64_t obs_write_note(const void* writer, const void* p, size_t bytes);
+bool obs_written_by_other(const void* reader, const void* p, size_t bytes, uint64_t since);
+void obs_write_forget(const void* writer);
 
 Family* make_mortar(int variant, int num_envs);
 Family* make_spot(int endless, int num_envs);
diff --git a/endless-memory-gym_amd/csrc/mg_mortar.hip b/endless-memory-gym_amd/csrc/mg_mortar.hip
--- a/endless-memory-gym_amd/csrc/mg_mortar.hip
+++ b/endless-memory-gym_amd/csrc/mg_mortar.hip
@@ -90,6 +90,63 @@
         if (dp->ring_on) stamp(R, STAMP_RING, dp->ring_x, dp->ring_y);
     }
 };
+
+constexpr uint32_t pack_box(int x0, int y0, int x1, int y1) {
+    return (uint32_t)x0 | (uint32_t)y0 << 8 | (uint32_t)x1 << 16 | (uint32_t)y1 << 24;
+}
+__device__ __forceinline__ bool same_frame(const uint32_t a[3], const uint32_t b[4]) {
+    return a[0] == b[0] && a[1] == b[1] && ((a[2] ^ b[2]) & 0xFFFFu) == 0u;
+}
+struct DirtySet {
+    uint32_t b[5];
+    static __device__ __forceinline__ uint32_t box(int x0, int y0, int w, int h) {
+        const int x1 = min(x0 + w, SCREEN), y1 = min(y0 + h, SCREEN);
+        x0 = max(x0, 0);
+        y0 = max(y0, 0);
+        return x0 < x1 && y0 < y1 ? pack_box(x0, y0, x1, y1) : 0u;
+    }
+    __device__ __forceinline__ void build(const MortarDesc& o, const MortarDesc& d, const AtlasTables* T, uint32_t tbox) {
+        b[0] = o.tmpl != d.tmpl ? tbox : 0u;
+        b[1] = b[2] = b[3] = b[4] = 0u;
+        if (o.sprite != d.sprite || o.sx != d.sx || o.sy != d.sy) {
+            if (o.sprite != 0xFF) { const StampInfo si = T->stamps[STAMP_SPRITE0 + o.sprite]; b[1] = box(o.sx, o.sy, si.w, si.h); }
+            if (d.sprite != 0xFF) { const StampInfo si = T->stamps[STAMP_SPRITE0 + d.sprite]; b[2] = box(d.sx, d.sy, si.w, si.h); }
+        }
+        if (o.glyph != d.glyph || o.glyph_x0 != d.glyph_x0) {
+            if (o.glyph < 9) { const StampInfo si = T->stamps[STAMP_GLYPH0 + o.glyph]; b[3] = box(o.glyph_x0, o.glyph_x0, si.w, si.h); }
+            if (d.glyph < 9) { const StampInfo si = T->stamps[STAMP_GLYPH0 + d.glyph]; b[4] = box(d.glyph_x0, d.glyph_x0, si.w, si.h); }
+        }
+    }
+    __device__ __forceinline__ void span(int& lo, int& hi) const {
+        lo = FRAME_BYTES;
+        hi = -1;
+#pragma unroll
+        for (int k = 0; k < 5; ++k) {
+            const int x0 = b[k] & 0xFF, y0 = (b[k] >> 8) & 0xFF, x1 = (b[k] >> 16) & 0xFF, y1 = b[k] >> 24;
+            if (b[k]) {
+                lo = min(lo, (x0 * SCREEN + y0) * 3);
+                hi = max(hi, ((x1 - 1) * SCREEN + y1) * 3 - 1);
+            }
+        }
+    }
+    __device__ __forceinline__ bool hits(int lo, int hi) const {
+        const int p0 = lo / 3, p1 = hi / 3, c0 = p0 / SCREEN, c1 = p1 / SCREEN;
+        const int ya = p0 - c0 * SCREEN, yb = c1 == c0 ? p1 - c0 * SCREEN : SCREEN - 1, yc = p1 - c1 * SCREEN;
+        bool hit = false;
+#pragma unroll
+        for (int k = 0; k < 5; ++k) {
+            const int x0 = b[k] & 0xFF, y0 = (b[k] >> 8) & 0xFF, x1 = (b[k] >> 16) & 0xFF, y1 = b[k] >> 24;
+            hit |= c0 >= x0 && c0 < x1 && ya < y1 && yb >= y0;
+            hit |= c1 != c0 && c1 >= x0 && c1 < x1 && yc >= y0;
+        }
+        return hit;
+    }
+};
+#ifdef MG_LAB_CHUNK_EXACT
+constexpr bool DIRTY_LINES = false;
+#else
+constexpr bool DIRTY_LINES = true;
+#endif
 
 constexpr uint32_t pack_deltas(const int (&v)[9]) {
     uint32_t m = 0;
@@ -532,7 +589,8 @@
 template <bool DONE_FLAG, bool FINAL = false>
 __global__ __launch_bounds__(256, 7) void mortar_step_raster_kernel(MortarStepArgs a, int logic_wgs, int logic_base, uint32_t epoch,
                                                                     uint32_t ticket, uint32_t* claims, uint32_t* rescues,
-                                                                    RasterAtlas A, void* __restrict__ obs, uint32_t* done_flag, uint32_t done_ticket) {
+                                                                    RasterAtlas A, void* __restrict__ obs, uint32_t* done_flag, uint32_t done_ticket,
+                                                                    MortarDesc* __restrict__ drawn, int full, uint32_t tbox) {
     const int n = a.n;
     const int tid = threadIdx.x, lane = tid & 63;
     const int rel = (int)blockIdx.x - logic_base;
@@ -559,22 +617,28 @@
     R.T = A.tables;
     R.tid = tid;
     const int stride = (int)gridDim.x - logic_wgs;
-    for (int v = (int)blockIdx.x < logic_base ? (int)blockIdx.x : (int)blockIdx.x - logic_wgs; v < n; v += stride) {
-        const int env = xcd_grouped_frame(v, n);
-        const uint32_t* src = reinterpret_cast<const uint32_t*>(a.io.desc + env);
-        uint32_t w[4];
-        bool tried = false;
+    const int v0 = (int)blockIdx.x < logic_base ? (int)blockIdx.x : (int)blockIdx.x - logic_wgs;
+    for (int vb = v0; vb < n; vb += 64 * stride) {
+        const int nb = min(64, (n - 1 - vb) / stride + 1);
+        const bool mine = lane < nb;
+        const int envl = mine ? xcd_grouped_frame(vb + lane * stride, n) : 0;
+        const uint32_t* srcl = reinterpret_cast<const uint32_t*>(a.io.desc + envl);
+        uint32_t w3l = 0u;
+        uint64_t tried = 0;
         unsigned long long t0 = 0;
         for (int polls = 0;; ++polls) {
-            w[3] = (uint32_t)__builtin_amdgcn_readfirstlane((int)__hip_atomic_load(src + 3, __ATOMIC_RELAXED, __HIP_MEMORY_SCOPE_AGENT));
-            if ((w[3] >> 24) == epoch) break;
+            if (mine) w3l = __hip_atomic_load(srcl + 3, __ATOMIC_RELAXED, __HIP_MEMORY_SCOPE_AGENT);
+            const uint64_t pending = __ballot(mine && (w3l >> 24) != epoch);
+            if (!pending) break;
 #if defined(MG_LABV) && MG_LABV >= 2
             if (false) {
 #else
             if (polls == 0) t0 = wall_clock64();
-            if (!tried && (polls & 15) == 15 && wall_clock64() - t0 >= RESCUE_AFTER_TICKS) {
+            if ((pending & ~tried) && (polls & 15) == 15 && wall_clock64() - t0 >= RESCUE_AFTER_TICKS) {
 #endif
-                tried = true;
+                const int first = __builtin_ctzll(pending & ~tried);
+                tried |= 1ull << first;
+                const int env = __builtin_amdgcn_readlane(envl, first);
                 if (claim(env >> 6)) {
                     const MortarStepArgs MG_KERNARG_AS* ka = (const MortarStepArgs MG_KERNARG_AS*)__builtin_amdgcn_kernarg_segment_ptr();
                     asm volatile("" : "+s"(ka));
@@ -588,9 +652,22 @@
             __builtin_amdgcn_s_sleep(4);
         }
         asm volatile("" ::: "memory");
-        w[0] = __hip_atomic_load(src + 0, __ATOMIC_RELAXED, __HIP_MEMORY_SCOPE_AGENT);
-        w[1] = __hip_atomic_load(src + 1, __ATOMIC_RELAXED, __HIP_MEMORY_SCOPE_AGENT);
-        w[2] = __hip_atomic_load(src + 2, __ATOMIC_RELAXED, __HIP_MEMORY_SCOPE_AGENT);
+        uint32_t wl[3] = {0u, 0u, 0u};
+        u32x4 ol = (u32x4)(0u);
+        if (mine) {
+#pragma unroll
+            for (int k = 0; k < 3; ++k) wl[k] = __hip_atomic_load(srcl + k, __ATOMIC_RELAXED, __HIP_MEMORY_SCOPE_AGENT);
+            if (!full) ol = *reinterpret_cast<const u32x4*>(drawn + envl);
+        }
+      for (int j = 0; j < nb; ++j) {
+        const int env = xcd_grouped_frame(vb + j * stride, n);
+        uint32_t w[4], ow[3];
+#pragma unroll
+        for (int k = 0; k < 3; ++k) w[k] = (uint32_t)__builtin_amdgcn_readlane((int)wl[k], j);
+        w[3] = (uint32_t)__builtin_amdgcn_readlane((int)w3l, j);
+        ow[0] = (uint32_t)__builtin_amdgcn_readlane((int)ol.x, j);
+        ow[1] = (uint32_t)__builtin_amdgcn_readlane((int)ol.y, j);
+        ow[2] = (uint32_t)__builtin_amdgcn_readlane((int)ol.z, j);
         MortarDesc d;
         memcpy(&d, w, sizeof(d));
         if constexpr (FINAL) {
@@ -614,10 +691,67 @@
         int t = tid;
         asm volatile("" : "+v"(t));
         R.tid = t;
-        MortarComposer::compose(&d, R);
+        DirtySet D;
+        int span_lo = 0, span_hi = FRAME_BYTES - 1;
+        if (!full) {
+            if (same_frame(ow, w)) continue;
+            MortarDesc od;
+            memset(&od, 0, sizeof(od));
+            memcpy(&od, ow, sizeof(ow));
+            D.build(od, d, R.T, tbox);
+            D.span(span_lo, span_hi);
+            span_lo -= 64;
+            span_hi += 64;
+        }
+        if (full || span_hi - span_lo > FRAME_BYTES / 2) {
+            MortarComposer::compose(&d, R);
+            __syncthreads();
+            store_frame<MG_OBS_U8_XYC, false>(smem, obs, env, t);
+        } else {
+            uint8_t* const row = static_cast<uint8_t*>(obs) + (size_t)env * FRAME_BYTES;
+            const int head = (int)((reinterpret_cast<uintptr_t>(row) >> 4) & 3);
+            uint32_t dirty = 0;
+#pragma unroll
+            for (int j = 0; j < 6; ++j) {
+                const int k = t + 256 * j;
+                if (16 * k + 15 < span_lo || 16 * k > span_hi) continue;
+                int lo = 16 * k, hi = lo + 15;
+                if (DIRTY_LINES) {
+                    lo -= 16 * ((head + k) & 3);
+                    hi = lo + 63;
+                    lo = max(lo, 0);
+                    hi = min(hi, FRAME_BYTES - 1);
+                }
+                if (k < FRAME_VEC16 && D.hits(lo, hi)) dirty |= 1u << j;
+            }
+            const u32x4* tsrc = reinterpret_cast<const u32x4*>(R.A.templates + (size_t)d.tmpl * FRAME_BYTES);
+            u32x4* lds16 = reinterpret_cast<u32x4*>(smem);
+            u32x4 v[6];
+#pragma unroll
+            for (int j = 0; j < 6; ++j)
+                v[j] = (j < 5 || t < TAIL) ? tsrc[t + 256 * j] : (u32x4)(0u);
+#pragma unroll
+            for (int j = 0; j < 6; ++j)
+                if (dirty & (1u << j)) lds16[t + 256 * j] = v[j];
+            __syncthreads();
+            if (d.sprite != 0xFF) stamp(R, STAMP_SPRITE0 + d.sprite, d.sx, d.sy);
+            if (d.glyph < 9) {
+                __syncthreads();
+                stamp(R, STAMP_GLYPH0 + d.glyph, d.glyph_x0, d.glyph_x0);
+            }
+            __syncthreads();
+            u32x4* dst = reinterpret_cast<u32x4*>(row);
+#pragma unroll
+            for (int j = 5; j >= 0; --j)
+                if (dirty & (1u << j)) dst[t + 256 * j] = lds16[t + 256 * j];
+        }
+        if (t == 0) {
+            u32x4 rec;
+            rec.x = w[0]; rec.y = w[1]; rec.z = w[2]; rec.w = w[3];
+            *reinterpret_cast<u32x4*>(drawn + env) = rec;
+        }
         __syncthreads();
-        store_frame<MG_OBS_U8_XYC, false>(smem, obs, env, t);
-        __syncthreads();
+      }
     }
     if constexpr (DONE_FLAG) {
         __builtin_amdgcn_fence(__ATOMIC_RELEASE, "");
@@ -667,6 +801,19 @@
 }
 
 static const double SCALE = 0.25;
+
+static uint32_t template_difference_box(const std::vector<uint8_t>& t) {
+    const size_t count = t.size() / FRAME_BYTES;
+    int x0 = SCREEN, y0 = SCREEN, x1 = 0, y1 = 0;
+    for (size_t k = 1; k < count; ++k)
+        for (int x = 0; x < SCREEN; ++x)
+            for (int y = 0; y < SCREEN; ++y) {
+                const size_t p = (size_t)(x * SCREEN + y) * 3;
+                if (memcmp(&t[p], &t[k * FRAME_BYTES + p], 3) == 0) continue;
+                x0 = std::min(x0, x); y0 = std::min(y0, y); x1 = std::max(x1, x + 1); y1 = std::max(y1, y + 1);
+            }
+    return x0 < x1 ? pack_box(x0, y0, x1, y1) : 0u;
+}
 
 class MortarFamily : public Family {
    public:
@@ -700,6 +847,7 @@
         state_.alloc(n);
         cmds_.alloc((size_t)n * P_.cmd_cap);
         desc_.alloc(n);
+        drawn_.alloc(n);
         tdesc_.alloc(n);
         rng_.alloc(n);
         err_.alloc();
@@ -720,6 +868,7 @@
         MG_HIP(hipDeviceSynchronize());
         P_.cmd_cap = (int)v;
         cmds_.alloc((size_t)n_ * P_.cmd_cap);
+        frames_valid_ = false;
         for (size_t k = 1; k < opt_.size(); ++k) copy_geometry(opt_[k]->P, P_);
         copy_geometry(defaults_, P_);
         sets_dirty_ = true;
@@ -815,6 +964,7 @@
                 throw OptionError{-3, "command_count x (command_show_duration + command_show_delay) exceeds the 65,535 entries of this build's display schedule"};
         }
         if (seeds) seeded_ = true;
+        frames_valid_ = false;
         upload_sets(s);
         if (per_set())
             hipLaunchKernelGGL(mortar_reset_kernel<true>, dim3((n_ + 255) / 256), dim3(256), 0, s, P_, n_, io(), seeds, mask, gt_dim() ? gt : nullptr);
@@ -840,24 +990,36 @@
             const int logic_wgs = (n_ + 255) / 256;
             const int frames = n_ < raster_grid(n_) ? n_ : raster_grid(n_);
             static const bool logic_last = lab_int("MEMGYM_LAB_LOGIC_LAST", 0) != 0;
+            const bool single = flag_armed_ && n_ == 1;
+            const Family* self = this;
+            const int full = (single || !incremental_ || !frames_valid_ || obs != tracked_ ||
+                              obs_written_by_other(self, obs, (size_t)n_ * FRAME_BYTES, tracked_seq_)) ? 1 : 0;
+            frames_valid_ = false;
             prof.begin(1, s);
-            if (flag_armed_ && n_ == 1) {
+            if (single) {
                 hipLaunchKernelGGL(mortar_step_raster_kernel<true>, dim3(logic_wgs + frames), dim3(256), RASTER_LDS, s, sa, logic_wgs,
-                                   logic_last ? frames : 0, epoch_, ticket_, claims_.p, rescues_.p, atlas_->dev(), obs, flag_dev_, flag_ticket_);
+                                   logic_last ? frames : 0, epoch_, ticket_, claims_.p, rescues_.p, atlas_->dev(), obs, flag_dev_, flag_ticket_,
+                                   drawn_.p, 1, tbox_);
                 flag_armed_ = false;
             } else if (ib.final_obs_dev && autoreset) {
                 MortarStepArgs fa = sa;
                 fa.tdesc = tdesc_.p;
                 hipLaunchKernelGGL((mortar_step_raster_kernel<false, true>), dim3(logic_wgs + frames), dim3(256), RASTER_LDS, s, fa, logic_wgs,
-                                   logic_last ? frames : 0, epoch_, ticket_, claims_.p, rescues_.p, atlas_->dev(), obs, (uint32_t*)nullptr, 0u);
+                                   logic_last ? frames : 0, epoch_, ticket_, claims_.p, rescues_.p, atlas_->dev(), obs, (uint32_t*)nullptr, 0u,
+                                   drawn_.p, full, tbox_);
             } else {
                 hipLaunchKernelGGL(mortar_step_raster_kernel<false>, dim3(logic_wgs + frames), dim3(256), RASTER_LDS, s, sa, logic_wgs,
-                                   logic_last ? frames : 0, epoch_, ticket_, claims_.p, rescues_.p, atlas_->dev(), obs, (uint32_t*)nullptr, 0u);
+                                   logic_last ? frames : 0, epoch_, ticket_, claims_.p, rescues_.p, atlas_->dev(), obs, (uint32_t*)nullptr, 0u,
+                                   drawn_.p, full, tbox_);
             }
             MG_HIP(hipGetLastError());
             prof.end(1, s);
+            tracked_ = obs;
+            tracked_seq_ = obs_write_note(self, obs, (size_t)n_ * FRAME_BYTES);
+            frames_valid_ = incremental_ && !single;
             return;
         }
+        frames_valid_ = false;
         prof.begin(0, s);
         const int sb = step_block(256);
         if (per_set()) hipLaunchKernelGGL(mortar_step_kernel<true>, dim3((n_ + sb - 1) / sb), dim3(sb), 0, s, sa);
@@ -957,8 +1119,13 @@
             circle(ring_stamp, r, r, r, (int)(8 * SCALE), 6);
             atlas_->add_stamp(ring_stamp);
         }
-        atlas_->set_templates(build_mortar_templates(P_.N, SCALE, SCREEN));
+        {
+            std::vector<uint8_t> tm = build_mortar_templates(P_.N, SCALE, SCREEN);
+            tbox_ = template_difference_box(tm);
+            atlas_->set_templates(tm);
+        }
         atlas_->upload();
+        frames_valid_ = false;
         P_.glyph_x0 = (int)((SCREEN / 2) - std::floor(88 * SCALE / 2));
         dirty_ = false;
         for (size_t k = 1; k < opt_.size(); ++k) copy_geometry(opt_[k]->P, P_);
@@ -993,6 +1160,8 @@
     }
 
     void raster_only(void* obs, const uint8_t* only, hipStream_t s) override {
+        const uintptr_t lo = (uintptr_t)obs, t = (uintptr_t)tracked_, bytes = (uintptr_t)n_ * FRAME_BYTES * 4;
+        if (tracked_ && lo < t + bytes && t < lo + bytes) frames_valid_ = false;
         launch_raster<MortarComposer>(desc_.p, atlas_->dev(), obs, obs_format, n_, s, only);
         MG_HIP(hipGetLastError());
     }
@@ -1031,13 +1200,23 @@
     bool dirty_ = true, seeded_ = false;
 
    public:
-    void on_state_loaded() override { seeded_ = true; }
+    void on_state_loaded() override { seeded_ = true; frames_valid_ = false; }
+    void invalidate_frames() override { frames_valid_ = false; }
+    void set_incremental_frames(bool on) override {
+        incremental_ = on;
+        frames_valid_ = false;
+    }
 
    private:
     float* vec_ = nullptr;
     DevArray<MortarState> state_;
     DevArray<uint8_t> cmds_;
     DevArray<MortarDesc> desc_, tdesc_;
+    DevArray<MortarDesc> drawn_;
+    uint32_t tbox_ = 0;
+    const void* tracked_ = nullptr;
+    uint64_t tracked_seq_ = 0;
+    bool frames_valid_ = false, incremental_ = true;
     RngStore rng_;
     ErrorWord err_;
     DevArray<uint32_t> claims_, rescues_;
diff --git a/endless-memory-gym_amd/csrc/mg_placement.hip b/endless-memory-gym_amd/csrc/mg_placement.hip
--- a/endless-memory-gym_amd/csrc/mg_placement.hip
+++ b/endless-memory-gym_amd/csrc/mg_placement.hip
@@ -356,6 +356,7 @@
         mg::set_error("mg_store_probe: bad arguments");
         return -1;
     }
+    mg::obs_write_note(nullptr, buf, n_frames * 21168);
     if (pattern == 0) {
         const size_t nvec = n_frames * 1323;
         hipLaunchKernelGGL(store_probe_linear_kernel, dim3((unsigned)((nvec + 255) / 256)), dim3(256), 0, stream, (u32x4*)buf, nvec);
diff --git a/endless-memory-gym_amd/memory_gym_amd/__init__.py b/endless-memory-gym_amd/memory_gym_amd/__init__.py
--- a/endless-memory-gym_amd/memory_gym_amd/__init__.py
+++ b/endless-memory-gym_amd/memory_gym_amd/__init__.py
@@ -6,14 +6,15 @@
 
 
 def make(env_id, num_envs=None, device=None, render_mode=None, obs_format="u8_xyc", final_observation=False, obs_buffer=None,
-         obs_placement=None, ground_truth64=False, on_capacity="raise", capacity=None):
+         obs_placement=None, ground_truth64=False, on_capacity="raise", capacity=None, incremental_frames=True):
     if num_envs is None:
         if env_id not in envs.CLASSES:
             raise ValueError("unknown env id %r" % (env_id,))
         return envs.CLASSES[env_id](render_mode=render_mode, device=device, capacity=capacity)
     return VecMemoryGym(env_id, num_envs=num_envs, device=device, render_mode=render_mode, obs_format=obs_format,
                         final_observation=final_observation, obs_buffer=obs_buffer, obs_placement=obs_placement,
-                        ground_truth64=ground_truth64, on_capacity=on_capacity, capacity=capacity)
+                        ground_truth64=ground_truth64, on_capacity=on_capacity, capacity=capacity,
+                        incremental_frames=incremental_frames)
 
 
 def _register_with_gymnasium():
diff --git a/endless-memory-gym_amd/memory_gym_amd/_native.py b/endless-memory-gym_amd/memory_gym_amd/_native.py
--- a/endless-memory-gym_amd/memory_gym_amd/_native.py
+++ b/endless-memory-gym_amd/memory_gym_amd/_native.py
@@ -85,6 +85,9 @@
     L.mg_set_capacity.argtypes = [C.c_void_p, C.c_char_p, C.c_int64]
     L.mg_capacity.argtypes = [C.c_void_p, C.c_char_p]
     L.mg_capacity.restype = C.c_int64
+    if hasattr(L, "mg_invalidate_frames"):
+        L.mg_invalidate_frames.argtypes = [C.c_void_p]
+        L.mg_set_incremental_frames.argtypes = [C.c_void_p, C.c_int]
     if hasattr(L, "mg_debug_counter"):
         L.mg_debug_counter.argtypes = [C.c_void_p, C.c_char_p, C.POINTER(C.c_int64)]
     return L
diff --git a/endless-memory-gym_amd/memory_gym_amd/vec_env.py b/endless-memory-gym_amd/memory_gym_amd/vec_env.py
--- a/endless-memory-gym_amd/memory_gym_amd/vec_env.py
+++ b/endless-memory-gym_amd/memory_gym_amd/vec_env.py
@@ -101,7 +101,7 @@
                    "f16_chw": (2, torch.float16, (3, 84, 84)), "bf16_chw": (3, torch.bfloat16, (3, 84, 84))}
 
     def __init__(self, env_id, num_envs=1, device=None, render_mode=None, obs_format="u8_xyc", final_observation=False,
-                 obs_buffer=None, obs_placement=None, ground_truth64=False, on_capacity="raise", capacity=None):
+                 obs_buffer=None, obs_placement=None, ground_truth64=False, on_capacity="raise", capacity=None, incremental_frames=True):
         if env_id not in DEFAULTS:
             raise ValueError("unknown env id %r" % (env_id,))
         if obs_format not in self.OBS_FORMATS:
@@ -199,6 +199,10 @@
         self._truncated = self.capacity_u8.view(torch.bool) if self.capacity_u8 is not None else torch.zeros(N, dtype=torch.bool, device=dev)
         self._n_actions = self.num_envs * self.action_dim
         self._p_err = C.byref(self._err)
+        self.incremental_frames = bool(incremental_frames) and hasattr(_native.LIB, "mg_set_incremental_frames")
+        if hasattr(_native.LIB, "mg_set_incremental_frames"):
+            _native.check(_native.LIB.mg_set_incremental_frames(h, 1 if self.incremental_frames else 0), "mg_set_incremental_frames")
+        self._obs_version = -1
         self._bind_step()
 
     def _stream(self):
@@ -347,9 +351,16 @@
             info["final_observation"] = self.final_obs
         return self._obs(), self.reward, self._done_bool, self._truncated, info
 
+    def invalidate_frames(self):
+        if self.incremental_frames:
+            _native.check(_native.LIB.mg_invalidate_frames(self._h), "mg_invalidate_frames")
+
     def _launch_step(self, a):
+        if self.incremental_frames and self.obs._version != self._obs_version:
+            _native.check(_native.LIB.mg_invalidate_frames(self._h), "mg_invalidate_frames")
         rc = _native.LIB.mg_step(self._h, a.data_ptr(), self.obs.data_ptr(), self._p_reward, self._p_done, self._p_gt, self._p_info,
                                  1 if self.autoreset else 0, self._raw_stream())
+        self._obs_version = self.obs._version
         if rc != 0:
             _native.check(rc, "mg_step")
 
@@ -367,6 +378,7 @@
             raise ValueError("use_obs_buffer: need a contiguous tensor like env.obs")
         self.obs = tensor
         self._swapped = True
+        self.invalidate_frames()
         self._bind_step()
 
     def use_step_buffers(self, reward, done_u8):
diff --git a/include/memgym.h b/include/memgym.h
--- a/include/memgym.h
+++ b/include/memgym.h
@@ -61,6 +61,10 @@
 int mg_step(mg_env* env, const int32_t* actions_dev, void* obs_dev, float* reward_dev, uint8_t* done_dev,
             float* gt_dev, const mg_info_buffers* info, int autoreset, void* stream);
 
+int mg_invalidate_frames(mg_env* env);
+
+int mg_set_incremental_frames(mg_env* env, int on);
+
 int mg_ground_truth64(mg_env* env, double* gt64_dev, void* stream);
 
 typedef struct mg_single_io {
```

Result: faster. 454.5 million env steps/s (median of 6 runs) (+55.5%).
